# mir-group/nequip

Hardware: NVIDIA H100
Metric: atom-steps/sec (energy+forces) (higher is better)
Workload: dtype f32

## Files before the change

include/nqb.h:

```cpp
#ifndef NQB_H
#define NQB_H

#include <stddef.h>
#include <stdint.h>

#ifdef __cplusplus
extern "C" {
#endif

typedef struct CUstream_st* nqb_stream_t;
typedef struct nqb_plan nqb_plan;

typedef struct nqb_irrep {
  int32_t mul;
  int32_t l;
  int32_t p;
} nqb_irrep;

typedef struct nqb_instruction {
  int32_t i_in1;
  int32_t i_in2;
  int32_t i_out;
} nqb_instruction;

enum { NQB_F32 = 0, NQB_F64 = 1 };

int nqb_abi_version(void);
const char* nqb_last_error(void);

int nqb_plan_create(const nqb_irrep* in1, int n_in1, const nqb_irrep* in2, int n_in2,
                    const nqb_irrep* out, int n_out, const nqb_instruction* ins, int n_ins,
                    const char* spec_lib_path, nqb_plan** plan);
void nqb_plan_destroy(nqb_plan* plan);
int nqb_plan_dims(const nqb_plan* plan, int* d_in, int* s_dim, int* weight_numel, int* d_out);
int nqb_plan_signature(const nqb_plan* plan, char* buf, int buflen);

int nqb_csr_check_sorted(const int64_t* keys, int64_t E, int32_t* flag_dev, nqb_stream_t st);
int nqb_csr_from_sorted(const int64_t* sorted_keys, int64_t E, int64_t N, int64_t* row_ptr ,
                        nqb_stream_t st);

int nqb_tp_scatter_fwd(const nqb_plan* plan, int dtype, const void* x, const void* y, const void* w,
                       const int64_t* row_ptr, const int64_t* perm, const int64_t* src, int64_t N,
                       int64_t E, void* out, nqb_stream_t st);

int nqb_tp_scatter_bwd(const nqb_plan* plan, int dtype, const void* x, const void* y, const void* w,
                       const int64_t* row_ptr, const int64_t* perm, const int64_t* src,
                       const void* grad_out, int64_t N, int64_t E, void* grad_x, void* grad_y,
                       void* grad_w, int deterministic,
                       nqb_stream_t st);
int nqb_tp_scatter_gy_slices(const nqb_plan* plan, int dtype);
int nqb_segment_sum(int dtype, const void* rows , int D, const int64_t* perm, const int64_t* seg_ptr ,
                    int64_t N, void* out , nqb_stream_t st);

int nqb_sh_fwd(int lmax, const double* vec, int64_t E, int out_dtype, void* y, nqb_stream_t st);
int nqb_sh_bwd(int lmax, const double* vec, int64_t E, int out_dtype, const void* grad_y,
               double* grad_vec, nqb_stream_t st);

int nqb_tp_fused_slices(const nqb_plan* plan);
int nqb_tp_fused_fwd(const nqb_plan* plan, const float* x, const float* y, const float* h, int64_t ldh, int K,
                     const float* w2_prepared, const int64_t* row_ptr, const int64_t* src, int64_t N, int64_t E,
                     float* out, float* w_out, const int32_t* slice_cta0, int nctas, nqb_stream_t st);

int nqb_edge_embed_fwd(int lmax, int num_bessel, double r_max, double poly_p, double prefactor,
                       const double* pos, const int64_t* edge_index, const double* shift,
                       const double* cell, int64_t N, int64_t E, int out_dtype, double* vec, void* y,
                       void* emb, nqb_stream_t st);
int nqb_edge_embed_bwd(int lmax, int num_bessel, double r_max, double poly_p, double prefactor,
                       const double* vec, const int64_t* edge_index, int64_t N, int64_t E,
                       int out_dtype, const void* grad_y, const void* grad_emb, double* grad_pos,
                       double* grad_vec, nqb_stream_t st);

int nqb_zbl_fwd(const double* pos, const int64_t* edge_index, const double* shift, const double* cell,
                const double* vec, const int64_t* types, const double* table, int T, const int64_t* row_ptr,
                const int64_t* perm, int64_t N, int64_t E, double r_max, double poly_p, int cutoff_f32,
                double* e_atom, nqb_stream_t st);
int nqb_zbl_bwd(const double* pos, const int64_t* edge_index, const double* shift, const double* cell,
                const double* vec, const int64_t* types, const double* table, int T, int64_t N, int64_t E,
                double r_max, double poly_p, int cutoff_f32, const double* grad_e_atom, double* grad_pos,
                double* grad_vec, nqb_stream_t st);

int nqb_nl_bin(const double* pos, int64_t N, const double* cell_host, const double* inv_host, const int* pbc,
               const int* nbins, const int* search, const double* lo, const double* width, double r_max,
               double* wpos , int32_t* base , int64_t* bin , int32_t* cidx ,
               nqb_stream_t st);
int nqb_nl_count(int64_t N, const double* cell_host, const double* inv_host, const int* pbc, const int* nbins,
                 const int* search, double r_max, const double* wpos, const int32_t* cidx, const int64_t* order,
                 const int64_t* bin_start, int64_t* counts , nqb_stream_t st);
int nqb_nl_fill(int64_t N, int64_t E, const double* cell_host, const double* inv_host, const int* pbc, const int* nbins,
                const int* search, double r_max, const double* wpos, const int32_t* cidx, const int32_t* base,
                const int64_t* order, const int64_t* bin_start, const int64_t* row_ptr ,
                int64_t* edge_index , double* shifts , nqb_stream_t st);
int nqb_nl_pad(int64_t N, int64_t capacity, const int64_t* row_ptr, int64_t* row_ptr_pad, int64_t* num_edges,
               int32_t* overflow, nqb_stream_t st);
int nqb_nl_fill_capacity(int64_t N, int64_t capacity, const double* cell_host, const double* inv_host, const int* pbc,
                         const int* nbins, const int* search, double r_max, const double* wpos, const int32_t* cidx,
                         const int32_t* base, const int64_t* order, const int64_t* bin_start,
                         const int64_t* row_ptr_pad , const int32_t* overflow ,
                         const double* pad_shift_host, int64_t* edge_index ,
                         double* shifts , nqb_stream_t st);
int64_t nqb_nl_params_bytes(void);
int nqb_nl_params_pack(const double* cell_host, const double* inv_host, const int* pbc, const int* nbins,
                       const int* search, double r_max, const double* pad_shift_host, void* out_host);
int nqb_nl_bin_dp(const double* pos, int64_t N, const void* params_dev, double* wpos ,
                  int32_t* base , int64_t* bin , int32_t* cidx , nqb_stream_t st);
int nqb_nl_count_dp(int64_t N, const void* params_dev, const double* wpos, const int32_t* cidx, const int64_t* order,
                    const int64_t* bin_start, int64_t* counts , nqb_stream_t st);
int nqb_nl_fill_capacity_dp(int64_t N, int64_t capacity, const void* params_dev, const double* wpos,
                            const int32_t* cidx, const int32_t* base, const int64_t* order, const int64_t* bin_start,
                            const int64_t* row_ptr_pad , const int32_t* overflow ,
                            int64_t* edge_index , double* shifts ,
                            nqb_stream_t st);

int nqb_mlp_hidden_fwd(const float* emb, const float* W1s, int64_t E, int num_bessel, int hidden, float* h,
                       nqb_stream_t st);
int nqb_mlp_hidden_bwd(const float* emb, const float* W1s, const float* grad_h, int64_t E, int num_bessel,
                       int hidden, float* grad_emb, nqb_stream_t st);

int64_t nqb_gemm_prepared_floats(int K, int N);
int nqb_gemm_prepare(const float* B, int64_t ldb, int K, int N, int transposed, float scale, float* prepared,
                     nqb_stream_t st);
int nqb_gemm_grouped(const void* descs_dev, int ndesc, int ntiles_total, const int32_t* tile_ctas_dev,
                     int sched_ctas, const float* a_base, const float* prepared_base, float* c_base,
                     const float* rowscale_base, int64_t rs_ld, int64_t M, nqb_stream_t st);
int nqb_gemm_grouped_act(const void* descs_dev, int ndesc, int ntiles_total, const int32_t* tile_ctas_dev,
                         int sched_ctas, const float* a_base, const float* prepared_base, float* c_base,
                         const float* rowscale_base, int64_t rs_ld, int64_t M, float* aux_base, nqb_stream_t st);

int nqb_gate_fwd(int dtype, const void* x, int64_t N, int d_in, int d_out, const int32_t* src,
                 const int32_t* gate, const int32_t* kind, void* out, nqb_stream_t st);
int nqb_gate_bwd(int dtype, const void* x, const void* grad_out, int64_t N, int d_in, int d_out,
                 const int32_t* tab, void* grad_x, nqb_stream_t st);

int64_t nqb_launch_count(void);

#ifdef __cplusplus
}
#endif
#endif
```

nequip_b200/_capi.py:

```python
from __future__ import annotations

import ctypes as C
import os
from typing import Optional

from . import build

_lib: Optional[C.CDLL] = None


class NqbIrrep(C.Structure):
    _fields_ = [("mul", C.c_int32), ("l", C.c_int32), ("p", C.c_int32)]


class NqbInstruction(C.Structure):
    _fields_ = [("i_in1", C.c_int32), ("i_in2", C.c_int32), ("i_out", C.c_int32)]


_vp, _i64, _i32, _dbl = C.c_void_p, C.c_int64, C.c_int, C.c_double

SIGNATURES = {
    "nqb_abi_version": (_i32, []),
    "nqb_last_error": (C.c_char_p, []),
    "nqb_launch_count": (_i64, []),
    "nqb_plan_create": (
        _i32,
        [C.POINTER(NqbIrrep), _i32, C.POINTER(NqbIrrep), _i32, C.POINTER(NqbIrrep), _i32,
         C.POINTER(NqbInstruction), _i32, C.c_char_p, C.POINTER(_vp)],
    ),
    "nqb_plan_destroy": (None, [_vp]),
    "nqb_plan_dims": (_i32, [_vp, C.POINTER(_i32), C.POINTER(_i32), C.POINTER(_i32), C.POINTER(_i32)]),
    "nqb_plan_signature": (_i32, [_vp, C.c_char_p, _i32]),
    "nqb_csr_check_sorted": (_i32, [_vp, _i64, _vp, _vp]),
    "nqb_csr_from_sorted": (_i32, [_vp, _i64, _i64, _vp, _vp]),
    "nqb_tp_scatter_fwd": (_i32, [_vp, _i32, _vp, _vp, _vp, _vp, _vp, _vp, _i64, _i64, _vp, _vp]),
    "nqb_tp_scatter_bwd": (
        _i32, [_vp, _i32, _vp, _vp, _vp, _vp, _vp, _vp, _vp, _i64, _i64, _vp, _vp, _vp, _i32, _vp]),
    "nqb_tp_fused_slices": (_i32, [_vp]),
    "nqb_tp_fused_fwd": (_i32, [_vp, _vp, _vp, _vp, _i64, _i32, _vp, _vp, _vp, _i64, _i64, _vp, _vp, _vp, _i32, _vp]),
    "nqb_tp_scatter_gy_slices": (_i32, [_vp, _i32]),
    "nqb_segment_sum": (_i32, [_i32, _vp, _i32, _vp, _vp, _i64, _vp, _vp]),
    "nqb_nl_bin": (_i32, [_vp, _i64, _vp, _vp, _vp, _vp, _vp, _vp, _vp, _dbl, _vp, _vp, _vp, _vp, _vp]),
    "nqb_nl_count": (_i32, [_i64, _vp, _vp, _vp, _vp, _vp, _dbl, _vp, _vp, _vp, _vp, _vp, _vp]),
    "nqb_nl_fill": (_i32, [_i64, _i64, _vp, _vp, _vp, _vp, _vp, _dbl, _vp, _vp, _vp, _vp, _vp, _vp, _vp, _vp, _vp]),
    "nqb_nl_pad": (_i32, [_i64, _i64, _vp, _vp, _vp, _vp, _vp]),
    "nqb_nl_fill_capacity": (
        _i32, [_i64, _i64, _vp, _vp, _vp, _vp, _vp, _dbl, _vp, _vp, _vp, _vp, _vp, _vp, _vp, _vp, _vp, _vp, _vp]),
    "nqb_nl_params_bytes": (_i64, []),
    "nqb_nl_params_pack": (_i32, [_vp, _vp, _vp, _vp, _vp, _dbl, _vp, _vp]),
    "nqb_nl_bin_dp": (_i32, [_vp, _i64, _vp, _vp, _vp, _vp, _vp, _vp]),
    "nqb_nl_count_dp": (_i32, [_i64, _vp, _vp, _vp, _vp, _vp, _vp, _vp]),
    "nqb_nl_fill_capacity_dp": (_i32, [_i64, _i64, _vp, _vp, _vp, _vp, _vp, _vp, _vp, _vp, _vp, _vp, _vp]),
    "nqb_sh_fwd": (_i32, [_i32, _vp, _i64, _i32, _vp, _vp]),
    "nqb_sh_bwd": (_i32, [_i32, _vp, _i64, _i32, _vp, _vp, _vp]),
    "nqb_edge_embed_fwd": (
        _i32, [_i32, _i32, _dbl, _dbl, _dbl, _vp, _vp, _vp, _vp, _i64, _i64, _i32, _vp, _vp, _vp, _vp]),
    "nqb_edge_embed_bwd": (
        _i32, [_i32, _i32, _dbl, _dbl, _dbl, _vp, _vp, _i64, _i64, _i32, _vp, _vp, _vp, _vp, _vp]),
    "nqb_zbl_fwd": (
        _i32, [_vp, _vp, _vp, _vp, _vp, _vp, _vp, _i32, _vp, _vp, _i64, _i64, _dbl, _dbl, _i32, _vp, _vp]),
    "nqb_zbl_bwd": (
        _i32, [_vp, _vp, _vp, _vp, _vp, _vp, _vp, _i32, _i64, _i64, _dbl, _dbl, _i32, _vp, _vp, _vp, _vp]),
    "nqb_mlp_hidden_fwd": (_i32, [_vp, _vp, _i64, _i32, _i32, _vp, _vp]),
    "nqb_mlp_hidden_bwd": (_i32, [_vp, _vp, _vp, _i64, _i32, _i32, _vp, _vp]),
    "nqb_gemm_prepared_floats": (_i64, [_i32, _i32]),
    "nqb_gemm_prepare": (_i32, [_vp, _i64, _i32, _i32, _i32, C.c_float, _vp, _vp]),
    "nqb_gate_fwd": (_i32, [_i32, _vp, _i64, _i32, _i32, _vp, _vp, _vp, _vp, _vp]),
    "nqb_gate_bwd": (_i32, [_i32, _vp, _vp, _i64, _i32, _i32, _vp, _vp, _vp]),
    "nqb_gemm_grouped": (_i32, [_vp, _i32, _i32, _vp, _i32, _vp, _vp, _vp, _vp, _i64, _i64, _vp]),
    "nqb_gemm_grouped_act": (_i32, [_vp, _i32, _i32, _vp, _i32, _vp, _vp, _vp, _vp, _i64, _i64, _vp, _vp]),
}


def lib() -> C.CDLL:
    global _lib
    if _lib is None:
        path = os.environ.get("NQB_RUNTIME_LIB") or build.ensure_runtime()
        L = C.CDLL(path, mode=C.RTLD_GLOBAL)
        for name, (res, args) in SIGNATURES.items():
            fn = getattr(L, name)
            fn.restype = res
            fn.argtypes = args
        if L.nqb_abi_version() != 2:
            raise RuntimeError("libnqb.so ABI version mismatch")
        _lib = L
    return _lib


def check(rc: int, what: str = "") -> None:
    if rc != 0:
        msg = lib().nqb_last_error()
        raise RuntimeError(f"libnqb {what}: {msg.decode() if msg else 'error'} (rc={rc})")


def launch_count() -> int:
    return int(lib().nqb_launch_count())
```

nequip_b200/csrc/nqb_gemm.cu:

```cuda
#include <cuda_runtime.h>
#include <stdint.h>
#include <stdio.h>

#include "../../include/nqb.h"
#include "nqb_tc.cuh"

namespace {

constexpr int TM = 128;
constexpr int TN = 128;
constexpr int KC = 32;
constexpr int MW = 64;
constexpr int NWG = TM / MW;
constexpr int DEPTH = 2;
constexpr int RAW = DEPTH + 1;
constexpr int NLO = 2;
constexpr int BSLOTS = 4;
constexpr int SEG = 320 / KC;
constexpr int NTHREADS = NWG * 128;
constexpr int BLOCK_FLOATS = 2 * TN * KC;

struct GemmDesc {
  int64_t a_off, c_off, b_off, rs_off;
  int64_t lda, ldc, K, N;
  int64_t kchunks, ntiles, tile0, flags;
};

struct Smem {
  float b[BSLOTS][BLOCK_FLOATS];
  float araw[NWG][RAW][MW * KC];
  float alo[NWG][NLO][MW * KC];
  uint64_t b_full[BSLOTS], b_empty[BSLOTS];
};

__device__ __forceinline__ const GemmDesc* find_desc(const GemmDesc* d, int nd, int q) {
  int i = 0;
  while (i + 1 < nd && d[i + 1].tile0 <= q) ++i;
  return d + i;
}

struct Sched {
  int q, q_step, nq_total;
  int64_t m_start, m_step;
  __device__ Sched(int b, int G, int T, const int32_t* tile_ctas, int sched_ctas) {
    nq_total = T;
    if (tile_ctas != nullptr && G == sched_ctas) {
      q = T; q_step = T; m_start = 0; m_step = 1;
      for (int t = 0; t < T; ++t) {
        const int c0 = tile_ctas[2 * t], n = tile_ctas[2 * t + 1];
        if (b >= c0 && b < c0 + n) { q = t; m_start = b - c0; m_step = n; break; }
      }
    } else if (T <= G) {
      const int R = G / T;
      q = (b < T * R) ? (b % T) : T;
      q_step = T;
      m_start = b / T;
      m_step = R;
    } else {
      q = b; q_step = G; m_start = 0; m_step = 1;
    }
  }
};

struct WorkQ {
  const GemmDesc* d;
  int nt, kchunks, K, ncols;
  bool resident;
};
__device__ __forceinline__ void decode_q(const GemmDesc* descs, int ndesc, int q, WorkQ& w) {
  w.d = find_desc(descs, ndesc, q);
  w.nt = q - (int)w.d->tile0;
  w.kchunks = (int)w.d->kchunks;
  w.K = (int)w.d->K;
  w.ncols = min(TN, (int)w.d->N - w.nt * TN);
  w.resident = w.kchunks <= BSLOTS;
}

__device__ __forceinline__ void bar_wg(int wg) { asm volatile("bar.sync %0, 128;" ::"r"(1 + wg) : "memory"); }

template <bool ACT>
__global__ void __launch_bounds__(NTHREADS, 1)
k_gemm3x(const GemmDesc* __restrict__ descs, int ndesc, int ntiles_total, const int32_t* __restrict__ tile_ctas,
         int sched_ctas, const float* __restrict__ a_base, const float* __restrict__ b_base, float* __restrict__ c_base,
         const float* __restrict__ rs_base, int64_t rs_ld, int64_t M, float* __restrict__ aux_base) {
  extern __shared__ __align__(1024) uint8_t smem_raw[];
  Smem& S = *reinterpret_cast<Smem*>(smem_raw);
  const int tid = threadIdx.x, wg = tid >> 7, warp = (tid >> 5) & 3, lane = tid & 31;
  const int64_t mtiles = (M + TM - 1) / TM;

  if (tid == 0) {
    for (int s = 0; s < BSLOTS; ++s) { mbar_init(&S.b_full[s], 1); mbar_init(&S.b_empty[s], NWG * 4); }
    fence_barrier_init();
  }
  __syncthreads();
  const Sched sch(blockIdx.x, gridDim.x, ntiles_total, tile_ctas, sched_ctas);

  const int r8 = lane & 7, kq = lane >> 3;
  const int my_off = (2 * warp) * (KC / 4 * 32) + kq * 32 + r8 * 4;
  int pq = sch.q, ph_ = 0, pnh = 1, pK = 0;
  int64_t pmt = sch.m_start, plda = 0;
  const float* pA = nullptr;
  bool pvalid = pq < sch.nq_total && sch.m_start < mtiles;
  auto open_q = [&]() {
    WorkQ w;
    decode_q(descs, ndesc, pq, w);
    pA = a_base + w.d->a_off;
    plda = w.d->lda;
    pK = w.K;
    pnh = w.kchunks;
  };
  if (pvalid) open_q();
  uint32_t n_issued = 0;
  auto issue = [&]() {
    if (pvalid) {
      float* dst = S.araw[wg][n_issued % RAW] + my_off;
#pragma unroll
      for (int g = 0; g < 2; ++g) {
        const int64_t m = pmt * TM + wg * MW + warp * 16 + g * 8 + r8;
#pragma unroll
        for (int kh = 0; kh < 2; ++kh) {
          const int k = ph_ * KC + (kh * 4 + kq) * 4;
          const bool in = m < M && k < pK;
          const int64_t off = in ? m * plda + k : 0;
          cp_async16(dst + g * (KC / 4 * 32) + kh * 128, pA + off, in ? 16u : 0u);
        }
      }
      if (++ph_ == pnh) {
        ph_ = 0;
        pmt += sch.m_step;
        if (pmt >= mtiles) {
          pmt = sch.m_start;
          pq += sch.q_step;
          pvalid = pq < sch.nq_total;
          if (pvalid) open_q();
        }
      }
    }
    ++n_issued;
    cp_async_commit();
  };
#pragma unroll 1
  for (int j = 0; j < DEPTH; ++j) issue();

  uint32_t bused = 0, bpar_ld = 0;
  auto load_slot = [&](int slot, const float* src, uint32_t bytes) {
    if ((bused >> slot) & 1) mbar_wait(&S.b_empty[slot], ((bpar_ld >> slot) & 1) ^ 1);
    mbar_expect_tx(&S.b_full[slot], 2 * bytes);
    bulk_g2s(S.b[slot], src, bytes, &S.b_full[slot]);
    bulk_g2s(S.b[slot] + TN * KC, src + TN * KC, bytes, &S.b_full[slot]);
    bused |= 1u << slot;
    bpar_ld ^= 1u << slot;
  };
  uint32_t bpar = 0;

  constexpr uint32_t SBO = (KC / 4) * 128, LBO = 128;
  constexpr uint32_t A_STAGE = (MW * KC * sizeof(float)) >> 4;
  constexpr uint32_t B_SLOT = (BLOCK_FLOATS * sizeof(float)) >> 4, B_LO = (TN * KC * sizeof(float)) >> 4;
  const uint64_t dR0 = make_desc(smem_u32(S.araw[wg][0]), LBO, SBO);
  const uint64_t dL0 = make_desc(smem_u32(S.alo[wg][0]), LBO, SBO);
  const uint64_t dB0 = make_desc(smem_u32(S.b[0]), LBO, SBO);
  const int r0 = warp * 16 + (lane >> 2), c0 = 2 * (lane & 3);
  float hh[64], xx[64], acc[64];
  uint32_t i = 0;

  for (int q = sch.q; q < sch.nq_total; q += sch.q_step) {
    WorkQ w;
    decode_q(descs, ndesc, q, w);
    if (sch.m_start >= mtiles) continue;
    const GemmDesc* d = w.d;
    const int nseg = (w.kchunks + SEG - 1) / SEG;
    const int64_t nmt = (mtiles - 1 - sch.m_start) / sch.m_step + 1;
    const int64_t nload = w.resident ? w.kchunks : nmt * w.kchunks;
    const uint32_t bytes = (uint32_t)TN * KC * sizeof(float);
    const float* B = b_base + d->b_off + (int64_t)w.nt * w.kchunks * BLOCK_FLOATS;
    if (tid == 0)
      for (int64_t c = 0; c < min((int64_t)BSLOTS, nload); ++c) load_slot((int)c, B + (c % w.kchunks) * BLOCK_FLOATS, bytes);
    int64_t x = 0, xr = 0;
    auto release = [&](int64_t y) {
      const int slot = (int)(y % BSLOTS);
      if (lane == 0) mbar_arrive(&S.b_empty[slot]);
      if (tid == 0 && y + BSLOTS < nload) load_slot(slot, B + ((y + BSLOTS) % w.kchunks) * BLOCK_FLOATS, bytes);
    };
    const bool reduce = (d->flags & 5) != 0, skipz = (d->flags & 2) != 0;
    const int64_t ldc = d->ldc;
    float* C = c_base + d->c_off + (int64_t)w.nt * TN;
    [[maybe_unused]] const int act = ACT ? (int)(d->flags >> 3) & 7 : 0;
    [[maybe_unused]] float* X = ACT && (act & 6) ? aux_base + d->c_off + (int64_t)w.nt * TN : nullptr;
    bool first_mt = true;
    for (int64_t mt = sch.m_start; mt < mtiles; mt += sch.m_step) {
      for (int seg = 0; seg < nseg; ++seg) {
        const int h1 = min(w.kchunks, (seg + 1) * SEG);
        for (int h = seg * SEG; h < h1; ++h, ++i) {
          cp_async_wait<DEPTH - 1>();
          const float* raw = S.araw[wg][i % RAW] + my_off;
          float* lo = S.alo[wg][i % NLO] + my_off;
#pragma unroll
          for (int g = 0; g < 2; ++g)
#pragma unroll
            for (int kh = 0; kh < 2; ++kh) {
              const float4 t = *reinterpret_cast<const float4*>(raw + g * (KC / 4 * 32) + kh * 128);
              *reinterpret_cast<float4*>(lo + g * (KC / 4 * 32) + kh * 128) =
                  make_float4(tf32_lo(t.x), tf32_lo(t.y), tf32_lo(t.z), tf32_lo(t.w));
            }
          fence_proxy_async();
          bar_wg(wg);
          uint32_t slot;
          if (w.resident) {
            slot = h;
            if (first_mt) { mbar_wait(&S.b_full[slot], (bpar >> slot) & 1); bpar ^= 1u << slot; }
          } else {
            slot = (uint32_t)(x++ % BSLOTS);
            mbar_wait(&S.b_full[slot], (bpar >> slot) & 1);
            bpar ^= 1u << slot;
          }
          const uint64_t a_hi = dR0 + (uint64_t)((i % RAW) * A_STAGE), a_lo = dL0 + (uint64_t)((i % NLO) * A_STAGE);
          const uint64_t b_hi = dB0 + (uint64_t)(slot * B_SLOT), b_lo = b_hi + B_LO;
          const uint32_t fresh = (h == seg * SEG);
          wgmma_fence();
#pragma unroll
          for (int ks = 0; ks < KC / 8; ++ks) wgmma_tf32_m64n128(hh, a_hi + ks * 16, b_hi + ks * 16, !(fresh && ks == 0));
#pragma unroll
          for (int ks = 0; ks < KC / 8; ++ks) wgmma_tf32_m64n128(xx, a_lo + ks * 16, b_hi + ks * 16, !(fresh && ks == 0));
#pragma unroll
          for (int ks = 0; ks < KC / 8; ++ks) wgmma_tf32_m64n128(xx, a_hi + ks * 16, b_lo + ks * 16, 1u);
          wgmma_commit();
          wgmma_wait<1>();
          if (xr + 1 < x) release(xr++);
          issue();
        }
        wgmma_wait<0>();
        if (xr < x) release(xr++);
        if (seg + 1 < nseg) {
#pragma unroll
          for (int j = 0; j < 64; ++j) acc[j] = (seg == 0 ? 0.f : acc[j]) + (hh[j] + xx[j]);
        } else {
#pragma unroll
          for (int j = 0; j < 64; ++j) hh[j] = (seg == 0) ? hh[j] + xx[j] : acc[j] + (hh[j] + xx[j]);
        }
      }
      const int64_t m0 = mt * TM + wg * MW + r0;
#pragma unroll
      for (int half = 0; half < 2; ++half) {
        const int64_t m = m0 + half * 8;
        float rs = 1.0f;
        if (d->rs_off >= 0) rs = (m < M) ? __ldg(rs_base + d->rs_off * rs_ld + m) : 0.f;
        if (m >= M || (skipz && rs == 0.f)) continue;
        float* crow = C + m * ldc + c0;
#pragma unroll
        for (int j = 0; j < TN / 8; ++j) {
          if (j * 8 + c0 < w.ncols) {
            float v0 = hh[4 * j + 2 * half] * rs, v1 = hh[4 * j + 2 * half + 1] * rs;
            if constexpr (ACT) {
              if (act != 0) {
                float* xp = X + m * ldc + c0 + j * 8;
                if (act & 4) {
                  const float2 p = *reinterpret_cast<const float2*>(xp);
                  const float s0 = sigmoid(p.x), s1 = sigmoid(p.y);
                  v0 *= s0 * fmaf(p.x, 1.0f - s0, 1.0f);
                  v1 *= s1 * fmaf(p.y, 1.0f - s1, 1.0f);
                } else {
                  if (act & 2) *reinterpret_cast<float2*>(xp) = make_float2(v0, v1);
                  if (act & 1) {
                    v0 *= sigmoid(v0);
                    v1 *= sigmoid(v1);
                  }
                }
              }
            }
            if (reduce)
              asm volatile("red.global.add.v2.f32 [%0], {%1, %2};" ::"l"(crow + j * 8), "f"(v0), "f"(v1) : "memory");
            else
              *reinterpret_cast<float2*>(crow + j * 8) = make_float2(v0, v1);
          }
        }
      }
      first_mt = false;
    }
    if (w.resident && lane == 0)
      for (int c = 0; c < w.kchunks; ++c) mbar_arrive(&S.b_empty[c]);
  }
  cp_async_wait<0>();
}

__global__ void k_gemm_prepare(const float* __restrict__ B, int64_t ldb, int K, int N, int transposed, float scale,
                               float* __restrict__ out, int kchunks, int ntiles) {
  const int64_t total = (int64_t)ntiles * kchunks * TN * KC;
  for (int64_t idx = (int64_t)blockIdx.x * blockDim.x + threadIdx.x; idx < total; idx += (int64_t)gridDim.x * blockDim.x) {
    const int kk = (int)(idx % KC);
    const int nn = (int)((idx / KC) % TN);
    const int64_t blk = idx / (KC * TN);
    const int c = (int)(blk % kchunks), j = (int)(blk / kchunks);
    const int k = c * KC + kk, n = j * TN + nn;
    float v = 0.f;
    if (k < K && n < N) v = (transposed ? B[(int64_t)n * ldb + k] : B[(int64_t)k * ldb + n]) * scale;
    const float hi = tf32_rn(v), lo = v - hi;
    float* tile = out + blk * BLOCK_FLOATS;
    const int off = canon_off(nn, kk, KC / 4);
    tile[off] = hi;
    tile[TN * KC + off] = lo;
  }
}

}

extern "C" int nqb_set_error(const char* msg);
extern "C" void nqb_count_launch(void);

static int gemm_device() {
  int dev = 0;
  cudaGetDevice(&dev);
  return dev & 63;
}
static int gemm_sm_count() {
  static int n[64] = {0};
  const int dev = gemm_device();
  if (n[dev] == 0) {
    cudaDeviceGetAttribute(&n[dev], cudaDevAttrMultiProcessorCount, dev);
    if (n[dev] <= 0) n[dev] = 132;
  }
  return n[dev];
}

extern "C" int64_t nqb_gemm_prepared_floats(int K, int N) {
  const int64_t kchunks = (K + KC - 1) / KC, ntiles = (N + TN - 1) / TN;
  return kchunks * ntiles * BLOCK_FLOATS;
}

extern "C" int nqb_gemm_prepare(const float* B, int64_t ldb, int K, int N, int transposed, float scale, float* prepared,
                                nqb_stream_t st) {
  if (!B || !prepared) return nqb_set_error("nqb_gemm_prepare: null pointer");
  if (K <= 0 || N <= 0) return nqb_set_error("nqb_gemm_prepare: bad shape");
  const int kchunks = (K + KC - 1) / KC, ntiles = (N + TN - 1) / TN;
  const int64_t total = (int64_t)ntiles * kchunks * TN * KC;
  int blocks = (int)((total + 255) / 256);
  if (blocks > 4096) blocks = 4096;
  k_gemm_prepare<<<blocks, 256, 0, (cudaStream_t)st>>>(B, ldb, K, N, transposed, scale, prepared, kchunks, ntiles);
  nqb_count_launch();
  cudaError_t e = cudaGetLastError();
  if (e != cudaSuccess) return nqb_set_error(cudaGetErrorString(e));
  return 0;
}

template <bool ACT>
static int gemm_grouped_launch(const char* who, const void* descs_dev, int ndesc, int ntiles_total,
                               const int32_t* tile_ctas_dev, int sched_ctas, const float* a_base,
                               const float* prepared_base, float* c_base, float* aux_base, const float* rowscale_base,
                               int64_t rs_ld, int64_t M, nqb_stream_t st) {
  auto fail = [&](const char* what) {
    char msg[160];
    snprintf(msg, sizeof(msg), "%s: %s", who, what);
    return nqb_set_error(msg);
  };
  if (ndesc <= 0 || ntiles_total <= 0) return fail("empty problem list");
  if (M < 0) return fail("negative M");
  if (M == 0) return 0;
  if (!descs_dev || !a_base || !prepared_base || !c_base) return fail("null pointer");
  if (ACT && !aux_base) return fail("aux_base is null (bit4 / bit5 problems store to or read from it)");
  if (((uintptr_t)a_base | (uintptr_t)prepared_base | (uintptr_t)c_base | (uintptr_t)aux_base) & 15)
    return fail(ACT ? "a_base, prepared_base, c_base and aux_base must be 16-byte aligned"
                    : "a_base, prepared_base and c_base must be 16-byte aligned");
  static bool attr_set[64] = {false};
  const int dev = gemm_device();
  if (!attr_set[dev]) {
    cudaError_t e = cudaFuncSetAttribute(k_gemm3x<ACT>, cudaFuncAttributeMaxDynamicSharedMemorySize, (int)sizeof(Smem) + 1024);
    if (e != cudaSuccess) return nqb_set_error(cudaGetErrorString(e));
    attr_set[dev] = true;
  }
  const int64_t nwork = ((M + TM - 1) / TM) * (int64_t)ntiles_total;
  int grid = (int)(nwork < gemm_sm_count() ? nwork : gemm_sm_count());
  if (tile_ctas_dev != nullptr && sched_ctas > 0 && sched_ctas <= gemm_sm_count()) grid = sched_ctas;
  else tile_ctas_dev = nullptr;
  k_gemm3x<ACT><<<grid, NTHREADS, sizeof(Smem) + 1024, (cudaStream_t)st>>>(
      (const GemmDesc*)descs_dev, ndesc, ntiles_total, tile_ctas_dev, sched_ctas, a_base, prepared_base, c_base,
      rowscale_base, rs_ld, M, aux_base);
  nqb_count_launch();
  cudaError_t e = cudaGetLastError();
  if (e != cudaSuccess) return nqb_set_error(cudaGetErrorString(e));
  return 0;
}

extern "C" int nqb_gemm_grouped(const void* descs_dev, int ndesc, int ntiles_total, const int32_t* tile_ctas_dev,
                                int sched_ctas, const float* a_base, const float* prepared_base, float* c_base,
                                const float* rowscale_base, int64_t rs_ld, int64_t M, nqb_stream_t st) {
  return gemm_grouped_launch<false>("nqb_gemm_grouped", descs_dev, ndesc, ntiles_total, tile_ctas_dev, sched_ctas,
                                    a_base, prepared_base, c_base, nullptr, rowscale_base, rs_ld, M, st);
}

extern "C" int nqb_gemm_grouped_act(const void* descs_dev, int ndesc, int ntiles_total, const int32_t* tile_ctas_dev,
                                    int sched_ctas, const float* a_base, const float* prepared_base, float* c_base,
                                    const float* rowscale_base, int64_t rs_ld, int64_t M, float* aux_base,
                                    nqb_stream_t st) {
  return gemm_grouped_launch<true>("nqb_gemm_grouped_act", descs_dev, ndesc, ntiles_total, tile_ctas_dev, sched_ctas,
                                   a_base, prepared_base, c_base, aux_base, rowscale_base, rs_ld, M, st);
}
```

nequip_b200/csrc/nqb_mlp.cu:

```cuda
#include <cuda_runtime.h>
#include <stdint.h>

#include "../../include/nqb.h"
#include "nqb_tc.cuh"

namespace {

constexpr int H = 128;
constexpr int NB = 8;

struct Basis8 { float4 a, b; };
__device__ __forceinline__ Basis8 load_basis(const float* __restrict__ emb, int64_t e, int64_t E) {
  Basis8 r;
  if (e < E) {
    r.a = __ldg(reinterpret_cast<const float4*>(emb + e * NB));
    r.b = __ldg(reinterpret_cast<const float4*>(emb + e * NB + 4));
  } else {
    r.a = make_float4(0.f, 0.f, 0.f, 0.f);
    r.b = r.a;
  }
  return r;
}
__device__ __forceinline__ void bcast_basis(const Basis8& mine, int j, float (&x)[NB]) {
  x[0] = __shfl_sync(0xffffffffu, mine.a.x, j); x[1] = __shfl_sync(0xffffffffu, mine.a.y, j);
  x[2] = __shfl_sync(0xffffffffu, mine.a.z, j); x[3] = __shfl_sync(0xffffffffu, mine.a.w, j);
  x[4] = __shfl_sync(0xffffffffu, mine.b.x, j); x[5] = __shfl_sync(0xffffffffu, mine.b.y, j);
  x[6] = __shfl_sync(0xffffffffu, mine.b.z, j); x[7] = __shfl_sync(0xffffffffu, mine.b.w, j);
}
__device__ __forceinline__ void preact4(const float (&x)[NB], const float2 (&w01)[NB], const float2 (&w23)[NB],
                                        float2& p01, float2& p23) {
  p01 = make_float2(0.f, 0.f);
  p23 = p01;
#pragma unroll
  for (int k = 0; k < NB; ++k) {
    const float2 xx = make_float2(x[k], x[k]);
    p01 = fma2_rn(xx, w01[k], p01);
    p23 = fma2_rn(xx, w23[k], p23);
  }
}

__global__ void __launch_bounds__(256) k_hidden_fwd(const float* __restrict__ emb, const float* __restrict__ W1s,
                                                    int64_t E, float* __restrict__ h) {
  const int lane = threadIdx.x & 31, m0 = lane * 4;
  float2 w01[NB], w23[NB];
#pragma unroll
  for (int k = 0; k < NB; ++k) {
    const float4 t = __ldg(reinterpret_cast<const float4*>(W1s + k * H + m0));
    w01[k] = make_float2(t.x, t.y);
    w23[k] = make_float2(t.z, t.w);
  }
  const int64_t nwarps = (int64_t)gridDim.x * (blockDim.x >> 5);
  const int64_t nbatch = (E + 31) >> 5;
  int64_t b = (int64_t)blockIdx.x * (blockDim.x >> 5) + (threadIdx.x >> 5);
  Basis8 cur = load_basis(emb, b * 32 + lane, b < nbatch ? E : 0);
  for (; b < nbatch; b += nwarps) {
    const int64_t bn = b + nwarps;
    const Basis8 nxt = load_basis(emb, bn * 32 + lane, bn < nbatch ? E : 0);
    const int64_t e0 = b * 32;
    const int cnt = (int)((E - e0) < 32 ? (E - e0) : 32);
    float* hrow = h + e0 * H + m0;
#pragma unroll 2
    for (int j = 0; j < cnt; ++j) {
      float x[NB];
      bcast_basis(cur, j, x);
      float2 p01, p23;
      preact4(x, w01, w23, p01, p23);
      float4 o;
      o.x = p01.x * sigmoid(p01.x);
      o.y = p01.y * sigmoid(p01.y);
      o.z = p23.x * sigmoid(p23.x);
      o.w = p23.y * sigmoid(p23.y);
      __stcs(reinterpret_cast<float4*>(hrow + (int64_t)j * H), o);
    }
    cur = nxt;
  }
}

__global__ void __launch_bounds__(256) k_hidden_bwd(const float* __restrict__ emb, const float* __restrict__ W1s,
                                                    const float* __restrict__ gh, int64_t E, float* __restrict__ gemb) {
  const int lane = threadIdx.x & 31, m0 = lane * 4;
  float2 w01[NB], w23[NB];
#pragma unroll
  for (int k = 0; k < NB; ++k) {
    const float4 t = __ldg(reinterpret_cast<const float4*>(W1s + k * H + m0));
    w01[k] = make_float2(t.x, t.y);
    w23[k] = make_float2(t.z, t.w);
  }
  const int64_t nwarps = (int64_t)gridDim.x * (blockDim.x >> 5);
  const int64_t nbatch = (E + 31) >> 5;
  int64_t b = (int64_t)blockIdx.x * (blockDim.x >> 5) + (threadIdx.x >> 5);
  Basis8 cur = load_basis(emb, b * 32 + lane, b < nbatch ? E : 0);
  for (; b < nbatch; b += nwarps) {
    const int64_t bn = b + nwarps;
    const Basis8 nxt = load_basis(emb, bn * 32 + lane, bn < nbatch ? E : 0);
    const int64_t e0 = b * 32;
    const int cnt = (int)((E - e0) < 32 ? (E - e0) : 32);
    const float* grow = gh + e0 * H + m0;
#pragma unroll 1
    for (int j0 = 0; j0 < cnt; j0 += 4) {
      float4 g[4];
#pragma unroll
      for (int u = 0; u < 4; ++u)
        g[u] = (j0 + u < cnt) ? __ldcs(reinterpret_cast<const float4*>(grow + (int64_t)(j0 + u) * H))
                              : make_float4(0.f, 0.f, 0.f, 0.f);
      float v[32];
#pragma unroll
      for (int u = 0; u < 4; ++u) {
        float x[NB];
        bcast_basis(cur, (j0 + u) & 31, x);
        float2 p01, p23;
        preact4(x, w01, w23, p01, p23);
        const float s0 = sigmoid(p01.x), s1 = sigmoid(p01.y), s2 = sigmoid(p23.x), s3 = sigmoid(p23.y);
        const float2 gp01 = make_float2(g[u].x * (s0 * fmaf(p01.x, 1.0f - s0, 1.0f)), g[u].y * (s1 * fmaf(p01.y, 1.0f - s1, 1.0f)));
        const float2 gp23 = make_float2(g[u].z * (s2 * fmaf(p23.x, 1.0f - s2, 1.0f)), g[u].w * (s3 * fmaf(p23.y, 1.0f - s3, 1.0f)));
#pragma unroll
        for (int k = 0; k < NB; ++k) {
          const float2 t = fma2_rn(gp23, w23[k], fmul2_rn(gp01, w01[k]));
          v[u * 8 + k] = t.x + t.y;
        }
      }
#define NQB_HALVE(O, C)                                                        \
  {                                                                            \
    const bool up = (lane & (O)) != 0;                                         \
    _Pragma("unroll") for (int j = 0; j < (C); ++j) {                          \
      const float mine = up ? v[j + (C)] : v[j];                               \
      const float theirs = up ? v[j] : v[j + (C)];                             \
      v[j] = mine + __shfl_xor_sync(0xffffffffu, theirs, (O));                 \
    }                                                                          \
  }
      NQB_HALVE(16, 16)
      NQB_HALVE(8, 8)
      NQB_HALVE(4, 4)
      NQB_HALVE(2, 2)
      NQB_HALVE(1, 1)
#undef NQB_HALVE
      if (j0 + (lane >> 3) < cnt) gemb[(e0 + j0) * NB + lane] = v[0];
    }
    cur = nxt;
  }
}

}

extern "C" int nqb_set_error(const char* msg);
extern "C" void nqb_count_launch(void);

template <typename K>
static unsigned hidden_grid(K kernel, int which, int64_t E) {
  static int ctas_dev[2][64] = {{0}, {0}};
  int dev = 0;
  cudaGetDevice(&dev);
  dev &= 63;
  if (ctas_dev[which][dev] == 0) {
    int sms = 0, occ = 0;
    cudaDeviceGetAttribute(&sms, cudaDevAttrMultiProcessorCount, dev);
    if (cudaOccupancyMaxActiveBlocksPerMultiprocessor(&occ, kernel, 256, 0) != cudaSuccess || occ <= 0) occ = 2;
    ctas_dev[which][dev] = (sms > 0 ? sms : 132) * occ;
  }
  const int64_t need = (((E + 31) >> 5) + 7) / 8;
  return (unsigned)(need < ctas_dev[which][dev] ? need : ctas_dev[which][dev]);
}

extern "C" int nqb_mlp_hidden_fwd(const float* emb, const float* W1s, int64_t E, int num_bessel, int hidden, float* h,
                                  nqb_stream_t st) {
  if (num_bessel != NB || hidden != H) return nqb_set_error("nqb_mlp_hidden_fwd: only num_bessel=8, hidden=128 is built");
  if (E < 0) return nqb_set_error("nqb_mlp_hidden_fwd: negative size");
  if (E == 0) return 0;
  if (!emb || !W1s || !h) return nqb_set_error("nqb_mlp_hidden_fwd: null pointer");
  k_hidden_fwd<<<hidden_grid(k_hidden_fwd, 0, E), 256, 0, (cudaStream_t)st>>>(emb, W1s, E, h);
  nqb_count_launch();
  cudaError_t e = cudaGetLastError();
  if (e != cudaSuccess) return nqb_set_error(cudaGetErrorString(e));
  return 0;
}

extern "C" int nqb_mlp_hidden_bwd(const float* emb, const float* W1s, const float* grad_h, int64_t E, int num_bessel,
                                  int hidden, float* grad_emb, nqb_stream_t st) {
  if (num_bessel != NB || hidden != H) return nqb_set_error("nqb_mlp_hidden_bwd: only num_bessel=8, hidden=128 is built");
  if (E < 0) return nqb_set_error("nqb_mlp_hidden_bwd: negative size");
  if (E == 0) return 0;
  if (!emb || !W1s || !grad_h || !grad_emb) return nqb_set_error("nqb_mlp_hidden_bwd: null pointer");
  k_hidden_bwd<<<hidden_grid(k_hidden_bwd, 1, E), 256, 0, (cudaStream_t)st>>>(emb, W1s, grad_h, E, grad_emb);
  nqb_count_launch();
  cudaError_t e = cudaGetLastError();
  if (e != cudaSuccess) return nqb_set_error(cudaGetErrorString(e));
  return 0;
}
```

nequip_b200/nn/dense.py:

```python
from __future__ import annotations

from typing import List, Optional, Tuple

import torch

from .. import ops
from ..irreps import Irreps


def _aligned(*vals) -> bool:
    return all(v % 4 == 0 for v in vals)


class _GemmLinearFn(torch.autograd.Function):
    @staticmethod
    def forward(ctx, x, fwd: ops.GroupedGemm, bwd: ops.GroupedGemm, d_out: int, zero_out: bool, d_in: int, zero_in: bool,
                rowscale, out_init):
        M = x.shape[0]
        if out_init is not None:
            out = out_init
        else:
            out = (torch.zeros if zero_out else torch.empty)((M, d_out), dtype=x.dtype, device=x.device)
        fwd.run(x, out, M, rowscale)
        ctx.bwd, ctx.d_in, ctx.zero_in, ctx.rowscale = bwd, d_in, zero_in, rowscale
        ctx.has_init = out_init is not None
        if out_init is not None:
            ctx.mark_dirty(out_init)
        return out

    @staticmethod
    @torch.autograd.function.once_differentiable
    def backward(ctx, gout):
        gout = gout.contiguous()
        M = gout.shape[0]
        gx = (torch.zeros if ctx.zero_in else torch.empty)((M, ctx.d_in), dtype=gout.dtype, device=gout.device)
        ctx.bwd.run(gout, gx, M, ctx.rowscale)
        return gx, None, None, None, None, None, None, None, (gout if ctx.has_init else None)


class IrrepsLinearGemm:

    def __init__(self, lin, device, extra_scale: float = 1.0, row_scaled: bool = False):
        fin, fout = lin.irreps_in, lin.irreps_out
        rs = 0 if row_scaled else -1
        self.row_scaled = row_scaled
        in_off, out_off = fin.offsets(), fout.offsets()
        self.d_in, self.d_out = fin.dim, fout.dim
        fwd: List[ops.GemmProblem] = []
        bwd: List[ops.GemmProblem] = []
        n_out = {o: sum(1 for (_, o2, _, _) in lin.instr if o2 == o) for o in range(len(fout))}
        n_in = {i: sum(1 for (i2, _, _, _) in lin.instr if i2 == i) for i in range(len(fin))}
        for (i, o, off, pw) in lin.instr:
            mi, ir = fin[i]
            mo = fout[o][0]
            W = lin.weight.detach()[off: off + mi * mo].view(mi, mo)
            for c in range(ir.dim):
                a_off, c_off = in_off[i] + c * mi, out_off[o] + c * mo
                fwd.append(ops.GemmProblem(a_off, self.d_in, c_off, self.d_out, W, scale=pw * extra_scale,
                                           atomic=n_out[o] > 1, rs_off=rs))
                bwd.append(ops.GemmProblem(c_off, self.d_out, a_off, self.d_in, W, scale=pw * extra_scale, transposed=True,
                                           atomic=n_in[i] > 1, rs_off=rs))
        self.zero_out = any(n != 1 for n in n_out.values())
        self.zero_in = any(n != 1 for n in n_in.values())
        self.fwd = ops.GroupedGemm(fwd, device)
        self.bwd = ops.GroupedGemm(bwd, device)

    @staticmethod
    def supported(lin) -> bool:
        muls = [m for m, _ in lin.irreps_in] + [m for m, _ in lin.irreps_out]
        return lin.layout == "ir_mul" and all(m % 4 == 0 for m in muls) and lin.weight.dtype == torch.float32

    def __call__(self, x, rowscale=None):
        if self.row_scaled != (rowscale is not None):
            raise ValueError("IrrepsLinearGemm: rowscale must be given exactly when built with row_scaled=True")
        return _GemmLinearFn.apply(x.contiguous(), self.fwd, self.bwd, self.d_out, self.zero_out, self.d_in, self.zero_in,
                                   rowscale, None)


class SelfConnectionGemm:

    def __init__(self, sc, type_table: torch.Tensor, device):
        fin, fout = sc.irreps_in, sc.irreps_out
        in_off, out_off = fin.offsets(), fout.offsets()
        self.d_in, self.d_out = fin.dim, fout.dim
        self.T = type_table.shape[0]
        fwd: List[ops.GemmProblem] = []
        bwd: List[ops.GemmProblem] = []
        tt = type_table.detach()
        for (i, o, off, pw) in sc.instr:
            mi, ir = fin[i]
            mo = fout[o][0]
            W = sc.weight.detach()[off: off + mi * sc.num_attr * mo].view(mi, sc.num_attr, mo)
            weff = torch.einsum("uvw,tv->tuw", W, tt)
            for t in range(self.T):
                for c in range(ir.dim):
                    a_off, c_off = in_off[i] + c * mi, out_off[o] + c * mo
                    multi_o = sum(1 for (_, o2, _, _) in sc.instr if o2 == o) > 1
                    fwd.append(ops.GemmProblem(a_off, self.d_in, c_off, self.d_out, weff[t].contiguous(), scale=pw,
                                               accumulate=not multi_o, atomic=multi_o, rs_off=t, skip_zero_rows=True))
                    multi_i = sum(1 for (i2, _, _, _) in sc.instr if i2 == i) > 1
                    bwd.append(ops.GemmProblem(c_off, self.d_out, a_off, self.d_in, weff[t].contiguous(), scale=pw,
                                               transposed=True, accumulate=not multi_i, atomic=multi_i, rs_off=t,
                                               skip_zero_rows=True))
        self.zero_in = True
        self.fwd = ops.GroupedGemm(fwd, device)
        self.bwd = ops.GroupedGemm(bwd, device)

    @staticmethod
    def supported(sc) -> bool:
        muls = [m for m, _ in sc.irreps_in] + [m for m, _ in sc.irreps_out]
        return sc.layout == "ir_mul" and all(m % 4 == 0 for m in muls) and sc.weight.dtype == torch.float32

    def __call__(self, x, types, base):
        onehot_t = torch.nn.functional.one_hot(types, self.T).to(x.dtype).t().contiguous()
        return _GemmLinearFn.apply(x.contiguous(), self.fwd, self.bwd, self.d_out, False, self.d_in, self.zero_in,
                                   onehot_t, base)


class _RadialMLPGemmFn(torch.autograd.Function):
    @staticmethod
    def forward(ctx, emb, mlp: "RadialMLPGemm", need_bwd: bool):
        E = emb.shape[0]
        out = torch.empty((E, mlp.W), dtype=emb.dtype, device=emb.device)
        pre = [] if need_bwd else None
        mlp.fwd.run(mlp.hidden(emb, pre), out, E)
        ctx.mlp = mlp
        if need_bwd:
            ctx.save_for_backward(emb, *pre)
        return out

    @staticmethod
    @torch.autograd.function.once_differentiable
    def backward(ctx, gw):
        emb, *pre = ctx.saved_tensors
        return ctx.mlp.grad_emb(emb, gw, pre), None, None


class RadialMLPGemm:

    def __init__(self, first, last, device, middle=()):
        self.w1s = (first.weight.detach() * first.alpha).contiguous()
        self.W = last.weight.shape[1]
        plan = self.plan(first, last, middle)
        self._hidden_kernel = plan["hidden_kernel"]

        def gemm(p):
            return ops.GroupedGemm([p], device)

        self.fwd = gemm(plan["fwd"])
        self.bwd = gemm(plan["bwd"])
        self._hidden = [(gemm(save), gemm(plain), save.B.shape[1]) for save, plain in plan["hidden"]]
        self._chain = [(self.bwd if p is plan["bwd"] else gemm(p), width, pre) for p, width, pre in plan["chain"]]

    @staticmethod
    def uses_hidden_kernel(first) -> bool:
        return tuple(first.weight.shape) == (8, 128)

    @classmethod
    def plan(cls, first, last, middle=()):

        def prob(lin, act="none", transposed=False):
            k, n = lin.weight.shape
            lda, ldc = (n, k) if transposed else (k, n)
            return ops.GemmProblem(0, lda, 0, ldc, lin.weight.detach(), scale=float(lin.alpha), transposed=transposed,
                                   act=act)

        layers = [first, *middle, last]
        kernel = cls.uses_hidden_kernel(first)
        skip = 1 if kernel else 0
        bwd = prob(last, transposed=True)
        chain = []
        for i in range(len(layers) - 1, 0, -1):
            pre = i - 1 - skip
            if pre >= 0:
                p = prob(layers[i], "silu_grad", True)
            else:
                p = bwd if i == len(layers) - 1 else prob(layers[i], transposed=True)
            chain.append((p, layers[i].weight.shape[0], pre if pre >= 0 else None))
        if not kernel:
            chain.append((prob(first, transposed=True), first.weight.shape[0], None))
        return dict(hidden_kernel=kernel, hidden=[(prob(l, "silu_save"), prob(l, "silu")) for l in layers[skip:-1]],
                    fwd=prob(last), bwd=bwd, chain=chain)

    @staticmethod
    def supported(first, last, dtype, middle=()) -> bool:
        dims = [first.weight.shape[0]] + [l.weight.shape[1] for l in (first, *middle, last)]
        return dtype == torch.float32 and all(d % 4 == 0 for d in dims)

    def hidden(self, emb, pre: Optional[list] = None):
        E = emb.shape[0]
        x = emb
        if self._hidden_kernel:
            x = torch.empty((E, self.w1s.shape[1]), dtype=emb.dtype, device=emb.device)
            ops.mlp_hidden_fwd(emb, self.w1s, x)
        for save, plain, width in self._hidden:
            h = torch.empty((E, width), dtype=emb.dtype, device=emb.device)
            if pre is None:
                plain.run(x, h, E)
            else:
                p = torch.empty((E, width), dtype=emb.dtype, device=emb.device)
                save.run(x, h, E, aux=p)
                pre.append(p)
            x = h
        return x

    def grad_emb(self, emb, gw, pre=()):
        E = emb.shape[0]
        g = gw.contiguous()
        for gemm, width, k in self._chain:
            out = torch.empty((E, width), dtype=g.dtype, device=g.device)
            gemm.run(g, out, E, aux=None if k is None else pre[k])
            g = out
        if self._hidden_kernel:
            gemb = torch.empty_like(emb)
            ops.mlp_hidden_bwd(emb, self.w1s, g, gemb)
            return gemb
        return g

    def __call__(self, emb):
        return _RadialMLPGemmFn.apply(emb.contiguous(), self, torch.is_grad_enabled() and emb.requires_grad)


class _FusedRadialTPFn(torch.autograd.Function):

    @staticmethod
    def forward(ctx, emb, x, y, edge_src, mod: "FusedRadialTP", csr, need_emb_grad: bool):
        pre = [] if need_emb_grad else None
        h = mod.mlp.hidden(emb, pre)
        need_bwd = any(ctx.needs_input_grad[:3])
        out, w = ops.tp_fused_fwd(mod.fw, x, y, h, edge_src, csr, want_w=need_bwd)
        ctx.mod, ctx.csr = mod, csr
        if need_bwd:
            ctx.save_for_backward(emb, x, y, w, edge_src, *(pre or ()))
        return out

    @staticmethod
    @torch.autograd.function.once_differentiable
    def backward(ctx, gout):
        emb, x, y, w, edge_src, *pre = ctx.saved_tensors
        mod = ctx.mod
        gx, gy, gw = ops.tp_scatter_bwd_raw(mod.plan, x, y, w, edge_src, ctx.csr, gout, need_x=ctx.needs_input_grad[1])
        gemb = mod.mlp.grad_emb(emb, gw, pre) if ctx.needs_input_grad[0] else None
        return gemb, gx, (gy if ctx.needs_input_grad[2] else None), None, None, None, None


class FusedRadialTP:

    def __init__(self, mlp: RadialMLPGemm, lin2, plan: ops.TPPlan, device):
        self.plan = plan
        self.mlp = mlp
        self.fw = ops.FusedTPWeights(plan, lin2.weight.detach(), float(lin2.alpha), device)

    @staticmethod
    def supported(lin1, lin2, plan: ops.TPPlan, dtype) -> bool:
        hid, W = lin2.weight.shape
        if dtype != torch.float32 or hid > 128 or hid % 8 or W != plan.weight_numel or W % 4:
            return False
        return int(ops._capi.lib().nqb_tp_fused_slices(plan.handle)) > 0

    def __call__(self, emb, x, y, edge_dst, edge_src):
        csr = ops.csr_cache.get(edge_dst.long().contiguous() if edge_dst.dtype != torch.int64 else edge_dst, x.shape[0])
        if csr.perm is not None:
            return None
        return _FusedRadialTPFn.apply(emb.contiguous(), x.contiguous(), y.contiguous(), edge_src.long().contiguous(), self, csr,
                                      torch.is_grad_enabled() and emb.requires_grad)
```

nequip_b200/nn/model.py:

```python
from __future__ import annotations

import math
from typing import Dict, List, Optional, Sequence, Tuple, Union

import torch

from .. import ops
from ..irreps import Irrep, Irreps, build_tp_instructions, tp_path_exists
from .pair import ZBL, ZBL_TARGET, parse_pair_potential
from .tp_scatter import B200TensorProductScatter

C_SILU = 1.6791767923989418
C_TANH = 1.5937334472592692

POSITIONS_KEY = "pos"
EDGE_INDEX_KEY = "edge_index"
EDGE_CELL_SHIFT_KEY = "edge_cell_shift"
CELL_KEY = "cell"
ATOM_TYPE_KEY = "atom_types"
TOTAL_ENERGY_KEY = "total_energy"
PER_ATOM_ENERGY_KEY = "atomic_energy"
FORCE_KEY = "forces"
STRESS_KEY = "stress"
VIRIAL_KEY = "virial"
EDGE_VECTORS_KEY = "edge_vectors"
EDGE_FORCE_KEY = "edge_forces"
BATCH_KEY = "batch"
BATCH_PTR_KEY = "ptr"
NUM_NODES_KEY = "num_atoms"


def feature_widths(l_max: int, num_features) -> List[int]:
    if isinstance(num_features, int):
        return [num_features] * (l_max + 1)
    widths = [int(f) for f in num_features]
    if len(widths) != l_max + 1:
        raise ValueError(f"num_features: expected an int or l_max + 1 = {l_max + 1} widths, got {list(num_features)}")
    return widths


def hidden_irreps(l_max: int, num_features, parity: bool) -> Irreps:
    widths = feature_widths(l_max, num_features)
    items = []
    for l in range(l_max + 1):
        ps = (1, -1) if parity else ((1,) if l % 2 == 0 else (-1,))
        for p in ps:
            items.append((widths[l], Irrep(l, p)))
    return Irreps(items)


def gate_irreps(prev: Irreps, edge_attr: Irreps, hidden: Irreps):
    scalars = Irreps([(mul, ir) for mul, ir in hidden if ir.l == 0 and tp_path_exists(prev, edge_attr, ir)])
    gated = Irreps([(mul, ir) for mul, ir in hidden if ir.l > 0 and tp_path_exists(prev, edge_attr, ir)])
    gate_ir = Irrep(0, 1) if tp_path_exists(prev, edge_attr, Irrep(0, 1)) else Irrep(0, -1)
    gates = Irreps([(mul, gate_ir) for mul, _ in gated])
    conv_out = (scalars + gates + gated).simplify()
    gated_out = Irreps([(mul, Irrep(ir.l, ir.p * gate_ir.p)) for mul, ir in gated])
    layer_out = scalars + gated_out
    return scalars, gates, gated, conv_out, layer_out


def layer_irreps(l_max: int, num_features, num_layers: int, parity: bool = True, type_embed_num_features=None):
    widths = feature_widths(l_max, num_features)
    f0 = type_embed_num_features or widths[0]
    edge_attr = Irreps.spherical_harmonics(l_max)
    prev = Irreps([(f0, Irrep(0, 1))])
    hid = hidden_irreps(l_max, widths, parity)
    hiddens = [hid] * (num_layers - 1) + [Irreps([(widths[0], Irrep(0, 1))])]
    out = []
    for h in hiddens:
        scalars, gates, gated, conv_out, layer_out = gate_irreps(prev, edge_attr, h)
        out.append((prev, edge_attr, conv_out, (scalars, gates, gated)))
        prev = layer_out
    return out


class ScalarLinearLayer(torch.nn.Module):

    def __init__(self, in_features: int, out_features: int, alpha: float = 1.0):
        super().__init__()
        self.in_features, self.out_features = in_features, out_features
        self.register_buffer("alpha", torch.tensor(alpha), persistent=False)
        self.weight = torch.nn.Parameter(torch.empty((in_features, out_features)))
        torch.nn.init.uniform_(self.weight, -math.sqrt(3), math.sqrt(3))

    def forward(self, x):
        return torch.mm(x, self.weight * self.alpha)


class ScalarMLPFunction(torch.nn.Module):

    def __init__(self, input_dim: int, output_dim: int, hidden_layers_depth: int = 0,
                 hidden_layers_width: Optional[int] = None, nonlinearity: Optional[str] = "silu"):
        super().__init__()
        dims = [input_dim] + hidden_layers_depth * [hidden_layers_width] + [output_dim]
        self.dims = dims
        layers: List[torch.nn.Module] = []
        nl = len(dims) - 1
        for layer, (h_in, h_out) in enumerate(zip(dims, dims[1:])):
            gain = 1.0 if nonlinearity is None or layer == 0 else math.sqrt(2)
            layers.append(ScalarLinearLayer(h_in, h_out, alpha=gain / math.sqrt(h_in)))
            if layer != nl - 1 and nonlinearity is not None:
                layers.append(torch.nn.SiLU())
        self.mlp = torch.nn.Sequential(*layers)

    def forward(self, x):
        return self.mlp(x)


class Linear(torch.nn.Module):

    def __init__(self, irreps_in, irreps_out, layout: str = "mul_ir"):
        super().__init__()
        self.layout = layout
        self.irreps_in, self.irreps_out = Irreps(irreps_in), Irreps(irreps_out)
        self.instr: List[Tuple[int, int, int, float]] = []
        off = 0
        pairs = [
            (i, o)
            for i, (_, ir_i) in enumerate(self.irreps_in)
            for o, (_, ir_o) in enumerate(self.irreps_out)
            if ir_i == ir_o
        ]
        for (i, o) in pairs:
            fan = sum(self.irreps_in[i2][0] for (i2, o2) in pairs if o2 == o)
            self.instr.append((i, o, off, 1.0 / math.sqrt(fan)))
            off += self.irreps_in[i][0] * self.irreps_out[o][0]
        self.weight_numel = off
        self.weight = torch.nn.Parameter(torch.randn(off))
        self._in_sl, self._out_sl = self.irreps_in.slices(), self.irreps_out.slices()

    def forward(self, x):
        N = x.shape[0]
        outs: List[Optional[torch.Tensor]] = [None] * len(self.irreps_out)
        for (i, o, off, pw) in self.instr:
            mi, ir = self.irreps_in[i]
            mo = self.irreps_out[o][0]
            W = self.weight[off: off + mi * mo].view(mi, mo) * pw
            if self.layout == "ir_mul":
                r = torch.matmul(x[:, self._in_sl[i]].reshape(N * ir.dim, mi), W).reshape(N, ir.dim * mo)
            else:
                xi = x[:, self._in_sl[i]].reshape(N, mi, ir.dim)
                r = torch.matmul(xi.transpose(1, 2), W).transpose(1, 2).reshape(N, mo * ir.dim)
            outs[o] = r if outs[o] is None else outs[o] + r
        for o, (mo, ir) in enumerate(self.irreps_out):
            if outs[o] is None:
                outs[o] = x.new_zeros(N, mo * ir.dim)
        return torch.cat(outs, dim=1)


class SelfConnection(torch.nn.Module):

    def __init__(self, irreps_in, num_attr: int, irreps_out, layout: str = "mul_ir"):
        super().__init__()
        self.layout = layout
        self.irreps_in, self.irreps_out, self.num_attr = Irreps(irreps_in), Irreps(irreps_out), num_attr
        pairs = [
            (i, o)
            for i, (_, ir_i) in enumerate(self.irreps_in)
            for o, (_, ir_o) in enumerate(self.irreps_out)
            if ir_i == ir_o
        ]
        self.instr: List[Tuple[int, int, int, float]] = []
        off = 0
        for (i, o) in pairs:
            fan = sum(self.irreps_in[i2][0] * num_attr for (i2, o2) in pairs if o2 == o)
            self.instr.append((i, o, off, 1.0 / math.sqrt(fan)))
            off += self.irreps_in[i][0] * num_attr * self.irreps_out[o][0]
        self.weight_numel = off
        self.weight = torch.nn.Parameter(torch.randn(off))
        self._in_sl = self.irreps_in.slices()

    def forward(self, x, node_attrs, types=None, type_table=None):
        N = x.shape[0]
        outs: List[Optional[torch.Tensor]] = [None] * len(self.irreps_out)
        fast = types is not None and type_table is not None
        if fast:
            T = type_table.shape[0]
            onehot = torch.nn.functional.one_hot(types, T).to(x.dtype)
        for (i, o, off, pw) in self.instr:
            mi, ir = self.irreps_in[i]
            mo = self.irreps_out[o][0]
            W = self.weight[off: off + mi * self.num_attr * mo].view(mi, self.num_attr, mo)
            if self.layout == "ir_mul":
                xk = x[:, self._in_sl[i]].reshape(N, ir.dim, mi)
                if fast:
                    weff = torch.einsum("uvw,tv->tuw", W, type_table).reshape(T * mi, mo) * pw
                    xe = (onehot.view(N, 1, T, 1) * xk.unsqueeze(2)).reshape(N * ir.dim, T * mi)
                    r = torch.matmul(xe, weff).reshape(N, ir.dim * mo)
                else:
                    r = pw * torch.einsum("uvw,nku,nv->nkw", W, xk, node_attrs).reshape(N, ir.dim * mo)
                outs[o] = r if outs[o] is None else outs[o] + r
                continue
            xi = x[:, self._in_sl[i]].reshape(N, mi, ir.dim)
            if fast:
                weff = torch.einsum("uvw,tv->tuw", W, type_table).reshape(T * mi, mo) * pw
                xe = (onehot.view(N, 1, T, 1) * xi.transpose(1, 2).unsqueeze(2)).reshape(N, ir.dim, T * mi)
                r = torch.matmul(xe, weff).transpose(1, 2).reshape(N, mo * ir.dim)
            else:
                r = pw * torch.einsum("uvw,nuk,nv->nwk", W, xi, node_attrs).reshape(N, mo * ir.dim)
            outs[o] = r if outs[o] is None else outs[o] + r
        for o, (mo, ir) in enumerate(self.irreps_out):
            if outs[o] is None:
                outs[o] = x.new_zeros(N, mo * ir.dim)
        return torch.cat(outs, dim=1)


class Gate(torch.nn.Module):

    def __init__(self, irreps_scalars, irreps_gates, irreps_gated, layout: str = "mul_ir"):
        super().__init__()
        self.layout = layout
        self.irreps_scalars, self.irreps_gates, self.irreps_gated = (
            Irreps(irreps_scalars), Irreps(irreps_gates), Irreps(irreps_gated))
        self.irreps_in = self.irreps_scalars + self.irreps_gates + self.irreps_gated
        gp = self.irreps_gates[0][1].p if len(self.irreps_gates) else 1
        self.irreps_out = self.irreps_scalars + Irreps([(m, Irrep(ir.l, ir.p * gp)) for m, ir in self.irreps_gated])
        self.use_fused = True
        self._tabs = None

    @staticmethod
    def _act(x, p: int):
        return torch.nn.functional.silu(x) * C_SILU if p == 1 else torch.tanh(x) * C_TANH

    def forward(self, x):
        if x.is_cuda and self.use_fused:
            key = (x.device, self.layout)
            if self._tabs is None or self._tabs[0] != key:
                self._tabs = (key, ops.GateTables(self.irreps_scalars, self.irreps_gates, self.irreps_gated,
                                                  self.layout, x.device))
            return ops.gate(x, self._tabs[1])
        N = x.shape[0]
        ns, ng = self.irreps_scalars.dim, self.irreps_gates.dim
        parts = []
        off = 0
        for mul, ir in self.irreps_scalars:
            parts.append(self._act(x[:, off: off + mul], ir.p))
            off += mul
        if len(self.irreps_gated):
            gates = []
            goff = ns
            for mul, ir in self.irreps_gates:
                gates.append(self._act(x[:, goff: goff + mul], ir.p))
                goff += mul
            gates = torch.cat(gates, dim=1)
            off = ns + ng
            g0 = 0
            for mul, ir in self.irreps_gated:
                if self.layout == "ir_mul":
                    ch = x[:, off: off + mul * ir.dim].reshape(N, ir.dim, mul)
                    parts.append((ch * gates[:, g0: g0 + mul].unsqueeze(1)).reshape(N, mul * ir.dim))
                else:
                    ch = x[:, off: off + mul * ir.dim].reshape(N, mul, ir.dim)
                    parts.append((ch * gates[:, g0: g0 + mul].unsqueeze(-1)).reshape(N, mul * ir.dim))
                off += mul * ir.dim
                g0 += mul
        return torch.cat(parts, dim=1)


class InteractionBlock(torch.nn.Module):

    def __init__(self, feature_irreps_in, irreps_edge_attr, feature_irreps_out, num_edge_embed: int,
                 num_node_attrs: int, radial_mlp_depth: int, radial_mlp_width: int, use_sc: bool,
                 avg_num_neighbors: float, is_first_layer: bool = False, layout: str = "mul_ir"):
        super().__init__()
        self.is_first_layer = is_first_layer
        self.layout = layout
        fin, fe, fout = Irreps(feature_irreps_in), Irreps(irreps_edge_attr), Irreps(feature_irreps_out)
        self.feature_irreps_in, self.irreps_edge_attr, self.feature_irreps_out = fin, fe, fout
        ann = [float(avg_num_neighbors)] if isinstance(avg_num_neighbors, (int, float)) else [float(v) for v in avg_num_neighbors]
        self.register_buffer("norm_const", torch.tensor([1.0 / math.sqrt(v) for v in ann]).reshape(-1, 1), persistent=False)
        self.norm_shortcut = len(ann) == 1
        self.linear_1 = Linear(fin, fin, layout)
        irreps_mid, instructions = build_tp_instructions(fin, fe, fout)
        self.irreps_mid, self.instructions = irreps_mid, instructions
        self.tp_scatter = B200TensorProductScatter(fin, fe, irreps_mid, instructions, layout=layout)
        self.edge_mlp = ScalarMLPFunction(num_edge_embed, self.tp_scatter.weight_numel,
                                          hidden_layers_depth=radial_mlp_depth,
                                          hidden_layers_width=radial_mlp_width, nonlinearity="silu")
        self.linear_2 = Linear(irreps_mid.simplify(), fout, layout)
        self.sc = SelfConnection(fin, num_node_attrs, fout, layout) if use_sc else None
        self.use_tensor_cores = True
        self.use_fused_radial_tp = "auto"
        self._fused_choice = None
        self.strict_fast_path = False
        self._tc_cache = None

    def _edge_weights(self, edge_embedding):
        return self.edge_mlp(edge_embedding)

    def _use_fused(self, tc, edge_embedding, x, edge_attrs, edge_index) -> bool:
        mode = self.use_fused_radial_tp
        if mode is True or mode is False:
            return mode
        if self._fused_choice is None:
            if torch.cuda.is_current_stream_capturing():
                return False
            with torch.no_grad():
                def t(fn):
                    fn()
                    torch.cuda.synchronize()
                    e0, e1 = torch.cuda.Event(enable_timing=True), torch.cuda.Event(enable_timing=True)
                    e0.record()
                    for _ in range(2):
                        fn()
                    e1.record()
                    torch.cuda.synchronize()
                    return e0.elapsed_time(e1) / 2

                xd, yd, ed = x.detach(), edge_attrs.detach(), edge_embedding.detach()
                tf = t(lambda: tc["fused"](ed, xd, yd, edge_index[0], edge_index[1]))
                tu = t(lambda: self.tp_scatter(x=xd, edge_attr=yd, edge_weight=tc["mlp"](ed), edge_dst=edge_index[0],
                                               edge_src=edge_index[1]))
            self._fused_choice = bool(tf < tu)
            self.fused_timing_ms = {"fused": tf, "unfused": tu}
        return self._fused_choice

    def _note_fallback(self, reason: str):
        if getattr(self, "strict_fast_path", False):
            raise RuntimeError(f"nequip_b200 InteractionBlock: tensor-core fast path unavailable ({reason}) and "
                               "strict_fast_path=True")
        seen = self.__dict__.setdefault("_fallback_seen", set())
        if reason not in seen:
            seen.add(reason)
            import warnings

            warnings.warn(f"nequip_b200 InteractionBlock: dense blocks run through torch.matmul (cuBLAS), not the "
                          f"wgmma kernels: {reason}", RuntimeWarning, stacklevel=3)

    def forward(self, x, node_attrs, edge_attrs, edge_embedding, edge_index, types=None, type_table=None,
                n_own: Optional[int] = None, halo=None):
        if n_own is not None and not self.is_first_layer:
            x = x[:n_own]
            node_attrs = node_attrs[:n_own]
            types = None if types is None else types[:n_own]
        tc = self._tensor_core_blocks(x, types, type_table)
        if tc is not None:
            x_in = x
            x = tc["lin1"](x) if self.norm_shortcut else tc["lin1"](x, self.norm_const.view(-1)[types].view(1, -1).contiguous())
            if halo is not None and not self.is_first_layer:
                x = halo(x)
            if tc["fused"] is not None and self._use_fused(tc, edge_embedding, x, edge_attrs, edge_index):
                y = tc["fused"](edge_embedding, x, edge_attrs, edge_index[0], edge_index[1])
                if y is not None:
                    x = y
                    if n_own is not None:
                        x = x[:n_own]
                    x = tc["lin2"](x)
                    if tc["sc"] is not None:
                        x = tc["sc"](x_in, types, x)
                    return x
            if tc["mlp"] is not None:
                w = tc["mlp"](edge_embedding)
            else:
                self._note_fallback("radial MLP shape not supported by the grouped GEMM (needs at least one hidden "
                                    "layer, num_bessels and widths multiples of 4)")
                w = self._edge_weights(edge_embedding)
            x = self.tp_scatter(x=x, edge_attr=edge_attrs, edge_weight=w, edge_dst=edge_index[0], edge_src=edge_index[1])
            if n_own is not None:
                x = x[:n_own]
            x = tc["lin2"](x)
            if tc["sc"] is not None:
                x = tc["sc"](x_in, types, x)
            return x
        sc = self.sc(x, node_attrs, types, type_table) if self.sc is not None else None
        x = self.linear_1(x)
        x = x * (self.norm_const.view(()) if self.norm_shortcut else self.norm_const[types])
        if halo is not None and not self.is_first_layer:
            x = halo(x)
        w = self._edge_weights(edge_embedding)
        x = self.tp_scatter(x=x, edge_attr=edge_attrs, edge_weight=w, edge_dst=edge_index[0], edge_src=edge_index[1])
        if n_own is not None:
            x = x[:n_own]
        x = self.linear_2(x)
        if sc is not None:
            x = x + sc
        return x

    def _tensor_core_blocks(self, x, types, type_table):
        from . import dense

        if not self.use_tensor_cores or not x.is_cuda:
            return None
        if x.dtype != torch.float32 or self.layout != "ir_mul":
            self._note_fallback(f"dtype {x.dtype} / layout {self.layout} (needs float32, ir_mul)")
            return None
        if any(p.requires_grad for p in self.parameters()) or (type_table is not None and type_table.requires_grad):
            self._note_fallback("parameters require grad (training); freeze them for the inference path")
            return None
        if (self.sc is not None or not self.norm_shortcut) and (types is None or type_table is None):
            self._note_fallback("self-connection / per-type normalisation need atom types + type table")
            return None
        key = tuple((p.data_ptr(), p._version) for p in self.parameters()) + (
            (type_table.data_ptr(), type_table._version) if type_table is not None else ())
        if self._tc_cache is not None and self._tc_cache[0] == key:
            if self._tc_cache[1] is None:
                self._note_fallback("a multiplicity is not a multiple of 4")
            return self._tc_cache[1]
        ok = dense.IrrepsLinearGemm.supported(self.linear_1) and dense.IrrepsLinearGemm.supported(self.linear_2)
        if self.sc is not None:
            ok = ok and dense.SelfConnectionGemm.supported(self.sc)
        if not ok:
            self._note_fallback("a multiplicity is not a multiple of 4")
            self._tc_cache = (key, None)
            return None
        dev = x.device
        lins = [m for m in self.edge_mlp.mlp if isinstance(m, ScalarLinearLayer)]
        mlp = fused = None
        if len(lins) >= 2 and dense.RadialMLPGemm.supported(lins[0], lins[-1], x.dtype, middle=lins[1:-1]):
            mlp = dense.RadialMLPGemm(lins[0], lins[-1], dev, middle=lins[1:-1])
            if dense.FusedRadialTP.supported(lins[0], lins[-1], self.tp_scatter._plan, x.dtype):
                fused = dense.FusedRadialTP(mlp, lins[-1], self.tp_scatter._plan, dev)
        blocks = dict(
            fused=fused,
            lin1=(dense.IrrepsLinearGemm(self.linear_1, dev, extra_scale=float(self.norm_const.view(-1)[0]))
                  if self.norm_shortcut else dense.IrrepsLinearGemm(self.linear_1, dev, row_scaled=True)),
            lin2=dense.IrrepsLinearGemm(self.linear_2, dev),
            sc=dense.SelfConnectionGemm(self.sc, type_table, dev) if self.sc is not None else None,
            mlp=mlp,
        )
        self._tc_cache = (key, blocks)
        return blocks


class ConvNetLayer(torch.nn.Module):

    def __init__(self, prev: Irreps, edge_attr: Irreps, hidden: Irreps, **conv_kwargs):
        super().__init__()
        scalars, gates, gated, conv_out, layer_out = gate_irreps(prev, edge_attr, hidden)
        self.equivariant_nonlin = Gate(scalars, gates, gated, conv_kwargs.get("layout", "mul_ir"))
        self.conv = InteractionBlock(prev, edge_attr, conv_out, **conv_kwargs)
        self.irreps_out = layer_out

    def forward(self, x, node_attrs, edge_attrs, edge_embedding, edge_index, types=None, type_table=None,
                n_own=None, halo=None):
        x = self.conv(x, node_attrs, edge_attrs, edge_embedding, edge_index, types, type_table, n_own, halo)
        return self.equivariant_nonlin(x)


NEQUIP_PRESETS: Dict[str, dict] = {
    "S": dict(num_layers=2, l_max=1, num_features=[128, 64]),
    "M": dict(num_layers=4, l_max=2, num_features=[128, 64, 32]),
    "L": dict(num_layers=6, l_max=3, num_features=[128, 64, 32, 32]),
    "XL": dict(num_layers=6, l_max=4, num_features=[320, 96, 64, 32, 32]),
}
NEQUIP_STANDARD_PRESET = dict(parity=False, type_embed_num_features=32, radial_mlp_depth=1, radial_mlp_width=128)


def preset_kwargs(name: str, **overrides) -> dict:
    key = name.upper()
    if key not in NEQUIP_PRESETS:
        raise ValueError(f"unknown preset {name!r}: expected one of {sorted(NEQUIP_PRESETS)}")
    return {**NEQUIP_STANDARD_PRESET, **NEQUIP_PRESETS[key], **overrides}


class NequIPEnergyModel(torch.nn.Module):

    def __init__(self, *, r_max: float, type_names: Sequence[str], num_layers: int = 4, l_max: int = 1,
                 parity: bool = True, num_features: Union[int, Sequence[int]] = 32,
                 type_embed_num_features: Optional[int] = None, radial_mlp_depth: int = 1,
                 radial_mlp_width: int = 128, num_bessels: int = 8, polynomial_cutoff_p: float = 6.0,
                 avg_num_neighbors: float = 1.0, per_type_energy_scales: Optional[Sequence[float]] = None,
                 per_type_energy_shifts: Optional[Sequence[float]] = None, model_dtype=torch.float32,
                 seed: int = 123, node_layout: str = "ir_mul", strict_fast_path: bool = False,
                 pair_potential: Optional[dict] = None):
        super().__init__()
        pair_spec = parse_pair_potential(pair_potential, len(type_names))
        widths = feature_widths(l_max, num_features)
        f_embed = int(type_embed_num_features) if type_embed_num_features is not None else widths[0]
        self.r_max, self.l_max, self.num_bessels, self.poly_p = float(r_max), l_max, num_bessels, float(polynomial_cutoff_p)
        self.model_dtype = model_dtype
        self.node_layout = node_layout
        self.config = dict(r_max=r_max, type_names=list(type_names), num_layers=num_layers, l_max=l_max, parity=parity,
                           num_features=num_features if isinstance(num_features, int) else widths,
                           type_embed_num_features=f_embed, radial_mlp_depth=radial_mlp_depth,
                           radial_mlp_width=radial_mlp_width, num_bessels=num_bessels,
                           polynomial_cutoff_p=polynomial_cutoff_p, avg_num_neighbors=avg_num_neighbors)
        prev_default = torch.get_default_dtype()
        torch.set_default_dtype(model_dtype)
        try:
            torch.manual_seed(seed)
            ntypes = len(type_names)
            if isinstance(avg_num_neighbors, dict):
                if set(avg_num_neighbors) != set(type_names):
                    raise ValueError("avg_num_neighbors: keys must be the type names")
                avg_num_neighbors = [float(avg_num_neighbors[k]) for k in type_names]
            elif not isinstance(avg_num_neighbors, (int, float)):
                avg_num_neighbors = [float(v) for v in avg_num_neighbors]
                if len(avg_num_neighbors) not in (1, ntypes):
                    raise ValueError(f"avg_num_neighbors: expected a scalar or {ntypes} values")
            self.config["avg_num_neighbors"] = avg_num_neighbors
            self.type_embed = torch.nn.Embedding(ntypes, f_embed)
            edge_attr = Irreps.spherical_harmonics(l_max)
            prev = Irreps([(f_embed, Irrep(0, 1))])
            hid = hidden_irreps(l_max, widths, parity)
            hiddens = [hid] * (num_layers - 1) + [Irreps([(widths[0], Irrep(0, 1))])]
            layers = []
            for li, h in enumerate(hiddens):
                layer = ConvNetLayer(prev, edge_attr, h, num_edge_embed=num_bessels, num_node_attrs=f_embed,
                                     radial_mlp_depth=radial_mlp_depth, radial_mlp_width=radial_mlp_width,
                                     use_sc=(li != 0), avg_num_neighbors=avg_num_neighbors,
                                     is_first_layer=(li == 0), layout=node_layout)
                layers.append(layer)
                prev = layer.irreps_out
            self.layers = torch.nn.ModuleList(layers)
            self.readout = ScalarMLPFunction(prev.dim, 1, hidden_layers_depth=0)
        finally:
            torch.set_default_dtype(prev_default)
        def table(v, what):
            if v is None:
                return torch.empty(0, dtype=torch.float64)
            t = torch.as_tensor(v, dtype=torch.float64).reshape(-1)
            if t.numel() == 1:
                t = t.expand(ntypes).clone()
            if t.numel() != ntypes:
                raise ValueError(f"{what}: expected a scalar or {ntypes} values (one per type), got {t.numel()}")
            return t.reshape(-1, 1)

        self.register_buffer("scales", table(per_type_energy_scales, "per_type_energy_scales"))
        self.register_buffer("shifts", table(per_type_energy_shifts, "per_type_energy_shifts"))
        self.pair_potential = None
        if pair_spec is not None:
            self.pair_potential = ZBL(type_names, model_dtype=model_dtype, **pair_spec)
            self.config["pair_potential"] = dict(_target_=ZBL_TARGET, **pair_spec)
        self.set_strict_fast_path(strict_fast_path)

    @classmethod
    def from_preset(cls, name: str, **kwargs) -> "NequIPEnergyModel":
        return cls(**preset_kwargs(name, **kwargs))

    def set_strict_fast_path(self, on: bool = True):
        for layer in self.layers:
            layer.conv.strict_fast_path = bool(on)
        return self

    @staticmethod
    def _reduce_energy(e_atom: torch.Tensor, data: Dict[str, torch.Tensor]) -> torch.Tensor:
        batch = data.get(BATCH_KEY)
        if batch is None:
            return e_atom.sum(dim=0, keepdim=True)
        if NUM_NODES_KEY in data:
            ng = int(data[NUM_NODES_KEY].numel())
        elif BATCH_PTR_KEY in data:
            ng = int(data[BATCH_PTR_KEY].numel()) - 1
        else:
            ng = int(batch.max().item()) + 1 if batch.numel() else 0
        out = torch.zeros((ng, 1), dtype=e_atom.dtype, device=e_atom.device)
        return out.index_add_(0, batch.view(-1).long(), e_atom)

    def energy(self, data: Dict[str, torch.Tensor]) -> Dict[str, torch.Tensor]:
        pos = data[POSITIONS_KEY]
        edge_index = data[EDGE_INDEX_KEY]
        types = data[ATOM_TYPE_KEY].view(-1)
        node_attrs = self.type_embed(types)
        x = node_attrs
        shift, cell = data.get(EDGE_CELL_SHIFT_KEY), data.get(CELL_KEY)
        if cell is None:
            shift = None
        pre = (2 * math.pi) / (self.r_max * self.r_max)
        sink = data.get("_edge_grad_sink")
        if EDGE_VECTORS_KEY in data:
            edge_attrs, edge_embedding = ops.edge_embed_from_vectors(
                data[EDGE_VECTORS_KEY], lmax=self.l_max, num_bessel=self.num_bessels, r_max=self.r_max,
                poly_p=self.poly_p, prefactor=pre, out_dtype=self.model_dtype)
        else:
            _vec, edge_attrs, edge_embedding = ops.edge_embed(
                pos, edge_index, shift, cell, lmax=self.l_max, num_bessel=self.num_bessels, r_max=self.r_max,
                poly_p=self.poly_p, prefactor=pre, out_dtype=self.model_dtype, edge_grad_sink=sink)
        for layer in self.layers:
            x = layer(x, node_attrs, edge_attrs, edge_embedding, edge_index, types, self.type_embed.weight)
        e_atom = self.readout(x).to(torch.float64)
        if self.scales.numel():
            e_atom = e_atom * self.scales[types]
        if self.shifts.numel():
            e_atom = e_atom + self.shifts[types]
        if self.pair_potential is not None:
            if EDGE_VECTORS_KEY in data:
                e_pair = self.pair_potential(types, edge_index, self.r_max, edge_vectors=data[EDGE_VECTORS_KEY])
            else:
                e_pair = self.pair_potential(types, edge_index, self.r_max, pos=pos, shift=shift, cell=cell,
                                             edge_grad_sink=sink)
            e_atom = e_atom + e_pair
        data[PER_ATOM_ENERGY_KEY] = e_atom
        data[TOTAL_ENERGY_KEY] = self._reduce_energy(e_atom, data)
        return data

    def energy_owned(self, data: Dict[str, torch.Tensor], n_own: int, halo) -> torch.Tensor:
        pos, edge_index = data[POSITIONS_KEY], data[EDGE_INDEX_KEY]
        types = data[ATOM_TYPE_KEY].view(-1)
        node_attrs = self.type_embed(types)
        x = node_attrs
        shift, cell = data.get(EDGE_CELL_SHIFT_KEY), data.get(CELL_KEY)
        if cell is None:
            shift = None
        _vec, edge_attrs, edge_embedding = ops.edge_embed(
            pos, edge_index, shift, cell, lmax=self.l_max, num_bessel=self.num_bessels, r_max=self.r_max,
            poly_p=self.poly_p, prefactor=(2 * math.pi) / (self.r_max * self.r_max), out_dtype=self.model_dtype)
        for layer in self.layers:
            x = layer(x, node_attrs, edge_attrs, edge_embedding, edge_index, types, self.type_embed.weight, n_own, halo)
        e_atom = self.readout(x).to(torch.float64)
        t_own = types[:n_own]
        if self.scales.numel():
            e_atom = e_atom * self.scales[t_own]
        if self.shifts.numel():
            e_atom = e_atom + self.shifts[t_own]
        if self.pair_potential is not None:
            e_atom = e_atom + self.pair_potential(types, edge_index, self.r_max, pos=pos, shift=shift, cell=cell)[:n_own]
        return e_atom

    def forward(self, data: Dict[str, torch.Tensor], compute_forces: bool = True,
                compute_stress: bool = False) -> Dict[str, torch.Tensor]:
        data = dict(data)
        if not compute_forces:
            return self.energy(data)
        if EDGE_VECTORS_KEY in data:
            with torch.enable_grad():
                vec = data[EDGE_VECTORS_KEY].detach().double().requires_grad_(True)
                data[EDGE_VECTORS_KEY] = vec
                data = self.energy(data)
                (g,) = torch.autograd.grad([data[TOTAL_ENERGY_KEY].sum()], [vec])
            data[EDGE_FORCE_KEY] = g
            data[EDGE_VECTORS_KEY] = vec.detach()
            data[TOTAL_ENERGY_KEY] = data[TOTAL_ENERGY_KEY].detach()
            data[PER_ATOM_ENERGY_KEY] = data[PER_ATOM_ENERGY_KEY].detach()
            return data
        if compute_stress and data.get(CELL_KEY) is None:
            raise ValueError("compute_stress needs a cell")
        pos = data[POSITIONS_KEY]
        sink = {} if compute_stress else None
        with torch.enable_grad():
            pos = pos.detach().requires_grad_(True)
            data[POSITIONS_KEY] = pos
            if sink is not None:
                data["_edge_grad_sink"] = sink
            data = self.energy(data)
            (g,) = torch.autograd.grad([data[TOTAL_ENERGY_KEY].sum()], [pos])
        data.pop("_edge_grad_sink", None)
        data[FORCE_KEY] = torch.neg(g)
        if sink is not None:
            g_edge = sink["edge_vector_grad"]
            if "pair_edge_vector_grad" in sink:
                g_edge = g_edge + sink["pair_edge_vector_grad"]
            v = torch.einsum("ea,eb->ab", sink["edge_vectors"], g_edge)
            v = 0.5 * (v + v.t())
            vol = torch.linalg.det(data[CELL_KEY].double().view(3, 3)).abs()
            data[STRESS_KEY] = (v / vol).view(1, 3, 3)
            data[VIRIAL_KEY] = torch.neg(v).view(1, 3, 3)
        data[POSITIONS_KEY] = pos.detach()
        data[TOTAL_ENERGY_KEY] = data[TOTAL_ENERGY_KEY].detach()
        data[PER_ATOM_ENERGY_KEY] = data[PER_ATOM_ENERGY_KEY].detach()
        return data
```

nequip_b200/ops.py:

```python
from __future__ import annotations

import ctypes as C
import os
import threading
from dataclasses import dataclass
from typing import Dict, List, Optional, Tuple

import torch

from . import _capi, build
from .codegen import GenOptions, TPSignature
from .irreps import Irreps

_DT = {torch.float32: 0, torch.float64: 1}


def _stream() -> int:
    return torch.cuda.current_stream().cuda_stream


def _ptr(t: Optional[torch.Tensor]) -> int:
    return 0 if t is None else t.data_ptr()


def _require_cuda(*ts: torch.Tensor):
    for t in ts:
        if t is not None and not t.is_cuda:
            raise RuntimeError(
                "nequip_b200 kernels run on CUDA (sm_90a) only; got a CPU tensor and there is no CPU fallback"
            )


class TPPlan:

    def __init__(self, irreps_in1, irreps_in2, irreps_out, instructions, opts: Optional[GenOptions] = None):
        self.sig = TPSignature(Irreps(irreps_in1), Irreps(irreps_in2), Irreps(irreps_out), list(instructions))
        self.opts = opts or GenOptions()
        self.spec_path = build.ensure_spec(self.sig, self.opts)
        L = _capi.lib()

        def arr(irr):
            a = (_capi.NqbIrrep * len(irr))()
            for i, (mul, ir) in enumerate(irr):
                a[i].mul, a[i].l, a[i].p = mul, ir.l, ir.p
            return a

        in1, in2, out = arr(self.sig.irreps_in1), arr(self.sig.irreps_in2), arr(self.sig.irreps_out)
        ins = (_capi.NqbInstruction * len(self.sig.instructions))()
        for i, (a, b, c) in enumerate(self.sig.instructions):
            ins[i].i_in1, ins[i].i_in2, ins[i].i_out = a, b, c
        h = C.c_void_p()
        _capi.check(
            L.nqb_plan_create(in1, len(in1), in2, len(in2), out, len(out), ins, len(ins),
                              self.spec_path.encode(), C.byref(h)),
            "nqb_plan_create",
        )
        self._h = h
        self.d_in, self.s_dim = self.sig.d_in, self.sig.s_dim
        self.weight_numel, self.d_out = self.sig.weight_numel, self.sig.d_out

    @property
    def handle(self) -> C.c_void_p:
        return self._h

    def __del__(self):
        try:
            if getattr(self, "_h", None):
                _capi.lib().nqb_plan_destroy(self._h)
                self._h = None
        except Exception:
            pass


_plans: Dict[str, TPPlan] = {}
_plans_lock = threading.Lock()


def get_plan(irreps_in1, irreps_in2, irreps_out, instructions, opts: Optional[GenOptions] = None) -> TPPlan:
    opts = opts or GenOptions()
    sig = TPSignature(Irreps(irreps_in1), Irreps(irreps_in2), Irreps(irreps_out), list(instructions))
    key = sig.canonical() + "|" + opts.tag()
    with _plans_lock:
        p = _plans.get(key)
        if p is None:
            p = TPPlan(irreps_in1, irreps_in2, irreps_out, instructions, opts)
            _plans[key] = p
        return p


@dataclass
class EdgeCSR:
    row_ptr: torch.Tensor
    perm: Optional[torch.Tensor]
    num_nodes: int
    num_edges: int


def build_csr(edge_dst: torch.Tensor, num_nodes: int, assume_sorted: Optional[bool] = None) -> EdgeCSR:
    _require_cuda(edge_dst)
    if edge_dst.dtype != torch.int64:
        edge_dst = edge_dst.long()
    edge_dst = edge_dst.contiguous()
    E = edge_dst.numel()
    L = _capi.lib()
    st = _stream()
    is_sorted = assume_sorted
    deferred = getattr(_sorted_tls, "flags", None)
    if deferred is None and _capture_flags and torch.cuda.is_current_stream_capturing():
        deferred = _capture_flags[-1]
    if is_sorted is None and deferred is not None:
        flag = torch.empty(1, dtype=torch.int32, device=edge_dst.device)
        _capi.check(L.nqb_csr_check_sorted(_ptr(edge_dst), E, _ptr(flag), st), "nqb_csr_check_sorted")
        deferred.append(flag)
        is_sorted = True
    if is_sorted is None:
        flag = torch.empty(1, dtype=torch.int32, device=edge_dst.device)
        _capi.check(L.nqb_csr_check_sorted(_ptr(edge_dst), E, _ptr(flag), st), "nqb_csr_check_sorted")
        is_sorted = bool(flag.item())
    perm = None
    keys = edge_dst
    if not is_sorted:
        keys, perm = torch.sort(edge_dst, stable=True)
        perm = perm.contiguous()
        keys = keys.contiguous()
    row_ptr = torch.empty(num_nodes + 1, dtype=torch.int64, device=edge_dst.device)
    _capi.check(L.nqb_csr_from_sorted(_ptr(keys), E, num_nodes, _ptr(row_ptr), st), "nqb_csr_from_sorted")
    return EdgeCSR(row_ptr, perm, num_nodes, E)


_sorted_tls = threading.local()
_capture_flags: List[List[torch.Tensor]] = []


class deferred_sorted_check:

    def __enter__(self):
        self.flags: List[torch.Tensor] = []
        self._prev = getattr(_sorted_tls, "flags", None)
        _sorted_tls.flags = self.flags
        _capture_flags.append(self.flags)
        return self

    def __exit__(self, *exc):
        _sorted_tls.flags = self._prev
        for k in range(len(_capture_flags) - 1, -1, -1):
            if _capture_flags[k] is self.flags:
                del _capture_flags[k]
                break
        return False


class _CSRCache:

    def __init__(self):
        self._tls = threading.local()

    def get(self, edge_dst: torch.Tensor, num_nodes: int) -> EdgeCSR:
        key = (edge_dst.data_ptr(), edge_dst.numel(), edge_dst._version, num_nodes, edge_dst.device)
        ent = getattr(self._tls, "ent", None)
        if ent is not None and ent[0] == key:
            return ent[1]
        csr = build_csr(edge_dst, num_nodes)
        self._tls.ent = (key, csr, edge_dst)
        return csr

    def clear(self):
        self._tls.ent = None


csr_cache = _CSRCache()


class _TPScatterFn(torch.autograd.Function):
    @staticmethod
    def forward(ctx, x, edge_attr, edge_weight, edge_src, plan: TPPlan, csr: EdgeCSR):
        L = _capi.lib()
        N, E = x.shape[0], edge_src.numel()
        out = torch.empty((N, plan.d_out), dtype=x.dtype, device=x.device)
        if N > 0:
            _capi.check(
                L.nqb_tp_scatter_fwd(plan.handle, _DT[x.dtype], _ptr(x), _ptr(edge_attr), _ptr(edge_weight),
                                     _ptr(csr.row_ptr), _ptr(csr.perm), _ptr(edge_src), N, E, _ptr(out), _stream()),
                "nqb_tp_scatter_fwd",
            )
        ctx.plan, ctx.csr = plan, csr
        ctx.save_for_backward(x, edge_attr, edge_weight, edge_src)
        return out

    @staticmethod
    @torch.autograd.function.once_differentiable
    def backward(ctx, gout):
        x, y, w, edge_src = ctx.saved_tensors
        gx, gy, gw = tp_scatter_bwd_raw(ctx.plan, x, y, w, edge_src, ctx.csr, gout, need_x=ctx.needs_input_grad[0])
        return gx, (gy if ctx.needs_input_grad[1] else None), (gw if ctx.needs_input_grad[2] else None), None, None, None


def tp_scatter(plan: TPPlan, x, edge_attr, edge_weight, edge_dst, edge_src, csr: Optional[EdgeCSR] = None):
    _require_cuda(x, edge_attr, edge_weight, edge_dst, edge_src)
    if x.dtype not in _DT:
        raise TypeError(f"nequip_b200.tp_scatter: unsupported dtype {x.dtype}")
    dt = x.dtype
    if x.dim() != 2 or x.shape[1] != plan.d_in:
        raise ValueError(f"x must be [N, {plan.d_in}], got {tuple(x.shape)}")
    E = edge_src.numel()
    if tuple(edge_attr.shape) != (E, plan.s_dim) or tuple(edge_weight.shape) != (E, plan.weight_numel):
        raise ValueError(
            f"edge_attr/edge_weight must be [{E}, {plan.s_dim}] / [{E}, {plan.weight_numel}], got "
            f"{tuple(edge_attr.shape)} / {tuple(edge_weight.shape)}"
        )
    if edge_dst.numel() != E:
        raise ValueError("edge_dst and edge_src differ in length")
    x = x.contiguous()
    y = edge_attr.to(dt).contiguous()
    w = edge_weight.to(dt).contiguous()
    src = edge_src.long().contiguous()
    if csr is None:
        csr = csr_cache.get(edge_dst.long().contiguous() if edge_dst.dtype != torch.int64 else edge_dst, x.shape[0])
    elif csr.num_nodes != x.shape[0] or csr.num_edges != E:
        raise ValueError("EdgeCSR does not match x / edge_index")
    return _TPScatterFn.apply(x, y, w, src, plan, csr)


class FusedTPWeights:

    def __init__(self, plan: TPPlan, W2: torch.Tensor, alpha2: float, device):
        from .codegen import TPGenerator

        L = _capi.lib()
        self.plan = plan
        lay = TPGenerator(plan.sig, plan.opts).fused_layout()
        nslice = int(L.nqb_tp_fused_slices(plan.handle))
        if lay is None or nslice == 0 or nslice != len(lay["slices"]):
            raise RuntimeError("FusedTPWeights: this signature has no fused kernel")
        K, W = int(W2.shape[0]), int(W2.shape[1])
        if W != plan.weight_numel or K > 128 or K % 8:
            raise ValueError(f"FusedTPWeights: W2 must be [K <= 128 (multiple of 8), {plan.weight_numel}], got {tuple(W2.shape)}")
        self.K, self.nslice = K, nslice
        cols = torch.tensor(lay["cols"], dtype=torch.long, device=device)
        W2d = W2.detach().to(device=device, dtype=torch.float32)
        Wp = torch.zeros((K, cols.numel()), dtype=torch.float32, device=device)
        ok = cols >= 0
        Wp[:, ok] = W2d[:, cols[ok]]
        self.prepared = self.prepare(Wp * float(alpha2), nslice)
        G = torch.cuda.get_device_properties(device).multi_processor_count
        self.cta0, self.nctas = self.split_grid(lay["cost"], G)
        self.cta0_dev = torch.tensor(self.cta0, dtype=torch.int32, device=device)

    @staticmethod
    def prepare(Wp: torch.Tensor, nslice: int) -> torch.Tensor:
        K = Wp.shape[0]
        wt = torch.zeros((nslice, 128, 128), dtype=torch.float32, device=Wp.device)
        wt[:, :, :K] = Wp.t().reshape(nslice, 128, K)
        bits = wt.view(torch.int32)
        hi = ((bits + 0x1000) & -0x2000).view(torch.float32)
        lo = wt - hi
        both = torch.stack([hi, lo], 1)
        both = both.reshape(nslice, 2, 16, 8, 32, 4).permute(0, 1, 2, 4, 3, 5)
        return both.contiguous().reshape(-1)

    @staticmethod
    def split_grid(cost, G: int):
        S = len(cost)
        n = [1] * S
        for _ in range(max(0, G - S)):
            i = max(range(S), key=lambda j: cost[j] / n[j])
            n[i] += 1
        pre = [0]
        for v in n:
            pre.append(pre[-1] + v)
        return pre, pre[-1]


def tp_fused_fwd(fw: FusedTPWeights, x: torch.Tensor, y: torch.Tensor, h: torch.Tensor, edge_src: torch.Tensor,
                 csr: EdgeCSR, want_w: bool):
    _require_cuda(x, y, h, edge_src)
    plan = fw.plan
    if csr.perm is not None:
        raise RuntimeError("tp_fused_fwd: edges must be grouped by destination (no permutation)")
    if x.dtype != torch.float32 or y.dtype != torch.float32 or h.dtype != torch.float32:
        raise TypeError("tp_fused_fwd: float32 only")
    N, E = x.shape[0], edge_src.numel()
    if x.shape[1] != plan.d_in or tuple(y.shape) != (E, plan.s_dim) or h.shape[0] != E or h.shape[1] != fw.K:
        raise ValueError("tp_fused_fwd: shape mismatch")
    x, y, h = x.contiguous(), y.contiguous(), h.contiguous()
    out = torch.empty((N, plan.d_out), dtype=torch.float32, device=x.device)
    w = torch.empty((E, plan.weight_numel), dtype=torch.float32, device=x.device) if want_w else None
    _capi.check(
        _capi.lib().nqb_tp_fused_fwd(plan.handle, _ptr(x), _ptr(y), _ptr(h), h.stride(0), fw.K, _ptr(fw.prepared),
                                     _ptr(csr.row_ptr), _ptr(edge_src), N, E, _ptr(out), _ptr(w), _ptr(fw.cta0_dev),
                                     int(fw.nctas), _stream()),
        "nqb_tp_fused_fwd",
    )
    return out, w


_DETERMINISTIC = os.environ.get("NQB_DETERMINISTIC", "0") not in ("", "0")


def set_deterministic(on: bool = True) -> None:
    global _DETERMINISTIC
    _DETERMINISTIC = bool(on)


def deterministic() -> bool:
    return _DETERMINISTIC or torch.are_deterministic_algorithms_enabled()


class _SrcCSRCache:

    def __init__(self):
        self._tls = threading.local()

    def get(self, edge_src: torch.Tensor, num_nodes: int):
        key = (edge_src.data_ptr(), edge_src.numel(), edge_src._version, num_nodes, edge_src.device)
        ent = getattr(self._tls, "ent", None)
        if ent is not None and ent[0] == key:
            return ent[1], ent[2]
        keys, perm = torch.sort(edge_src, stable=True)
        seg = torch.empty(num_nodes + 1, dtype=torch.int64, device=edge_src.device)
        _capi.check(_capi.lib().nqb_csr_from_sorted(_ptr(keys.contiguous()), edge_src.numel(), num_nodes, _ptr(seg), _stream()),
                    "nqb_csr_from_sorted")
        self._tls.ent = (key, perm.contiguous(), seg, edge_src)
        return self._tls.ent[1], seg

    def clear(self):
        self._tls.ent = None


src_csr_cache = _SrcCSRCache()


def tp_scatter_bwd_raw(plan: TPPlan, x, y, w, edge_src, csr: EdgeCSR, gout, need_x: bool = True,
                       force_deterministic: Optional[bool] = None):
    L = _capi.lib()
    N, E = x.shape[0], edge_src.numel()
    det = deterministic() if force_deterministic is None else bool(force_deterministic)
    gw = torch.empty_like(w)
    if N == 0 or E == 0:
        gw.zero_()
        return (torch.zeros_like(x) if need_x else None), torch.zeros_like(y), gw
    gout = gout.contiguous()
    dt = _DT[x.dtype]
    if not det:
        gx = torch.zeros_like(x) if need_x else None
        gy = torch.zeros_like(y)
        _capi.check(L.nqb_tp_scatter_bwd(plan.handle, dt, _ptr(x), _ptr(y), _ptr(w), _ptr(csr.row_ptr), _ptr(csr.perm),
                                         _ptr(edge_src), _ptr(gout), N, E, _ptr(gx), _ptr(gy), _ptr(gw), 0, _stream()),
                    "nqb_tp_scatter_bwd")
        return gx, gy, gw
    ns = int(L.nqb_tp_scatter_gy_slices(plan.handle, dt))
    if ns <= 0:
        raise RuntimeError("nequip_b200: this kernel library has no deterministic backward")
    gxe = torch.empty((E, x.shape[1]), dtype=x.dtype, device=x.device) if need_x else None
    gys = torch.zeros((ns, E, y.shape[1]), dtype=y.dtype, device=y.device)
    _capi.check(L.nqb_tp_scatter_bwd(plan.handle, dt, _ptr(x), _ptr(y), _ptr(w), _ptr(csr.row_ptr), _ptr(csr.perm),
                                     _ptr(edge_src), _ptr(gout), N, E, _ptr(gxe), _ptr(gys), _ptr(gw), 1, _stream()),
                "nqb_tp_scatter_bwd")
    gx = None
    if need_x:
        perm_t, seg_t = src_csr_cache.get(edge_src, N)
        gx = torch.empty_like(x)
        _capi.check(L.nqb_segment_sum(dt, _ptr(gxe), x.shape[1], _ptr(perm_t), _ptr(seg_t), N, _ptr(gx), _stream()),
                    "nqb_segment_sum")
    gy = gys[0]
    for q in range(1, ns):
        gy = gy + gys[q]
    return gx, gy, gw


class _SHFn(torch.autograd.Function):
    @staticmethod
    def forward(ctx, vec, lmax: int, out_dtype):
        L = _capi.lib()
        E = vec.shape[0]
        y = torch.empty((E, (lmax + 1) ** 2), dtype=out_dtype, device=vec.device)
        _capi.check(L.nqb_sh_fwd(lmax, _ptr(vec), E, _DT[out_dtype], _ptr(y), _stream()), "nqb_sh_fwd")
        ctx.lmax, ctx.out_dtype = lmax, out_dtype
        ctx.save_for_backward(vec)
        return y

    @staticmethod
    @torch.autograd.function.once_differentiable
    def backward(ctx, gy):
        (vec,) = ctx.saved_tensors
        L = _capi.lib()
        E = vec.shape[0]
        gvec = torch.empty_like(vec)
        gy = gy.to(ctx.out_dtype).contiguous()
        _capi.check(L.nqb_sh_bwd(ctx.lmax, _ptr(vec), E, _DT[ctx.out_dtype], _ptr(gy), _ptr(gvec), _stream()),
                    "nqb_sh_bwd")
        return gvec, None, None


def spherical_harmonics(vec: torch.Tensor, lmax: int, out_dtype=torch.float32) -> torch.Tensor:
    _require_cuda(vec)
    if vec.dim() != 2 or vec.shape[1] != 3:
        raise ValueError("vec must be [E, 3]")
    return _SHFn.apply(vec.double().contiguous(), int(lmax), out_dtype)


class _EdgeEmbedFn(torch.autograd.Function):
    @staticmethod
    def forward(ctx, pos, edge_index, shift, cell, lmax, num_bessel, r_max, poly_p, prefactor, out_dtype, sink=None):
        L = _capi.lib()
        N, E = pos.shape[0], edge_index.shape[1]
        dev = pos.device
        vec = torch.empty((E, 3), dtype=torch.float64, device=dev)
        y = torch.empty((E, (lmax + 1) ** 2), dtype=out_dtype, device=dev)
        emb = torch.empty((E, num_bessel), dtype=out_dtype, device=dev)
        _capi.check(
            L.nqb_edge_embed_fwd(lmax, num_bessel, r_max, poly_p, prefactor, _ptr(pos), _ptr(edge_index), _ptr(shift),
                                 _ptr(cell), N, E, _DT[out_dtype], _ptr(vec), _ptr(y), _ptr(emb), _stream()),
            "nqb_edge_embed_fwd",
        )
        ctx.args = (lmax, num_bessel, r_max, poly_p, prefactor, out_dtype, N)
        ctx.sink = sink
        ctx.save_for_backward(vec, edge_index)
        ctx.mark_non_differentiable(vec)
        return vec, y, emb

    @staticmethod
    @torch.autograd.function.once_differentiable
    def backward(ctx, _gvec, gy, gemb):
        vec, edge_index = ctx.saved_tensors
        lmax, num_bessel, r_max, poly_p, prefactor, out_dtype, N = ctx.args
        L = _capi.lib()
        E = vec.shape[0]
        gpos = torch.zeros((N, 3), dtype=torch.float64, device=vec.device)
        gy = None if gy is None else gy.to(out_dtype).contiguous()
        gemb = None if gemb is None else gemb.to(out_dtype).contiguous()
        gvec = torch.empty_like(vec) if ctx.sink is not None else None
        _capi.check(
            L.nqb_edge_embed_bwd(lmax, num_bessel, r_max, poly_p, prefactor, _ptr(vec), _ptr(edge_index), N, E,
                                 _DT[out_dtype], _ptr(gy), _ptr(gemb), _ptr(gpos), _ptr(gvec), _stream()),
            "nqb_edge_embed_bwd",
        )
        if ctx.sink is not None:
            ctx.sink["edge_vectors"], ctx.sink["edge_vector_grad"] = vec, gvec
        return gpos, None, None, None, None, None, None, None, None, None, None


class _EdgeEmbedVecFn(torch.autograd.Function):

    @staticmethod
    def forward(ctx, vec, lmax, num_bessel, r_max, poly_p, prefactor, out_dtype):
        L = _capi.lib()
        E = vec.shape[0]
        dev = vec.device
        pos = torch.cat([vec, torch.zeros((1, 3), dtype=torch.float64, device=dev)], 0)
        ar = torch.arange(E, dtype=torch.int64, device=dev)
        edge_index = torch.stack([torch.full_like(ar, E), ar]).contiguous()
        vec_out = torch.empty((E, 3), dtype=torch.float64, device=dev)
        y = torch.empty((E, (lmax + 1) ** 2), dtype=out_dtype, device=dev)
        emb = torch.empty((E, num_bessel), dtype=out_dtype, device=dev)
        _capi.check(
            L.nqb_edge_embed_fwd(lmax, num_bessel, r_max, poly_p, prefactor, _ptr(pos), _ptr(edge_index), 0, 0, E + 1, E,
                                 _DT[out_dtype], _ptr(vec_out), _ptr(y), _ptr(emb), _stream()),
            "nqb_edge_embed_fwd",
        )
        ctx.args = (lmax, num_bessel, r_max, poly_p, prefactor, out_dtype)
        ctx.save_for_backward(vec_out, edge_index)
        return y, emb

    @staticmethod
    @torch.autograd.function.once_differentiable
    def backward(ctx, gy, gemb):
        vec, edge_index = ctx.saved_tensors
        lmax, num_bessel, r_max, poly_p, prefactor, out_dtype = ctx.args
        E = vec.shape[0]
        gvec = torch.empty_like(vec)
        gy = None if gy is None else gy.to(out_dtype).contiguous()
        gemb = None if gemb is None else gemb.to(out_dtype).contiguous()
        _capi.check(
            _capi.lib().nqb_edge_embed_bwd(lmax, num_bessel, r_max, poly_p, prefactor, _ptr(vec), _ptr(edge_index), E + 1, E,
                                           _DT[out_dtype], _ptr(gy), _ptr(gemb), 0, _ptr(gvec), _stream()),
            "nqb_edge_embed_bwd",
        )
        return gvec, None, None, None, None, None, None


def edge_embed_from_vectors(vec, *, lmax: int, num_bessel: int = 8, r_max: float, poly_p: float = 6.0,
                            prefactor: float = 1.0, out_dtype=torch.float32):
    _require_cuda(vec)
    return _EdgeEmbedVecFn.apply(vec.double().contiguous(), int(lmax), int(num_bessel), float(r_max), float(poly_p),
                                 float(prefactor), out_dtype)


def edge_embed(pos, edge_index, shift=None, cell=None, *, lmax: int, num_bessel: int = 8, r_max: float,
               poly_p: float = 6.0, prefactor: float = 1.0, out_dtype=torch.float32, edge_grad_sink=None):
    _require_cuda(pos, edge_index)
    pos = pos.double().contiguous()
    edge_index = edge_index.long().contiguous()
    if (shift is None) != (cell is None):
        raise ValueError("shift and cell must be given together")
    if shift is not None:
        shift = shift.double().contiguous()
        cell = cell.double().reshape(3, 3).contiguous()
    return _EdgeEmbedFn.apply(pos, edge_index, shift, cell, int(lmax), int(num_bessel), float(r_max),
                              float(poly_p), float(prefactor), out_dtype, edge_grad_sink)


class _ZBLFn(torch.autograd.Function):
    @staticmethod
    def forward(ctx, geom, edge_index, shift, cell, types, table, r_max, poly_p, cutoff_f32, from_vectors, sink):
        N, E, T = types.numel(), edge_index.shape[1], table.shape[0]
        csr = csr_cache.get(edge_index[0], N)
        pos, vec = (None, geom) if from_vectors else (geom, None)
        e_atom = torch.empty((N, 1), dtype=torch.float64, device=types.device)
        _capi.check(
            _capi.lib().nqb_zbl_fwd(_ptr(pos), _ptr(edge_index), _ptr(shift), _ptr(cell), _ptr(vec), _ptr(types),
                                    _ptr(table), T, _ptr(csr.row_ptr), _ptr(csr.perm), N, E, r_max, poly_p,
                                    int(cutoff_f32), _ptr(e_atom), _stream()),
            "nqb_zbl_fwd",
        )
        ctx.args = (r_max, poly_p, cutoff_f32, from_vectors)
        ctx.sink = sink
        ctx.save_for_backward(geom, edge_index, shift, cell, types, table)
        return e_atom

    @staticmethod
    @torch.autograd.function.once_differentiable
    def backward(ctx, ge):
        geom, edge_index, shift, cell, types, table = ctx.saved_tensors
        r_max, poly_p, cutoff_f32, from_vectors = ctx.args
        N, E = types.numel(), edge_index.shape[1]
        pos, vec = (None, geom) if from_vectors else (geom, None)
        gpos = None if from_vectors else torch.zeros_like(geom)
        gvec = torch.empty((E, 3), dtype=torch.float64, device=geom.device) \
            if from_vectors or ctx.sink is not None else None
        ge = ge.to(torch.float64).contiguous()
        _capi.check(
            _capi.lib().nqb_zbl_bwd(_ptr(pos), _ptr(edge_index), _ptr(shift), _ptr(cell), _ptr(vec), _ptr(types),
                                    _ptr(table), table.shape[0], N, E, r_max, poly_p, int(cutoff_f32), _ptr(ge),
                                    _ptr(gpos), _ptr(gvec), _stream()),
            "nqb_zbl_bwd",
        )
        if ctx.sink is not None:
            ctx.sink["pair_edge_vector_grad"] = gvec
        return (gvec if from_vectors else gpos), None, None, None, None, None, None, None, None, None, None


def zbl_energy(pos, edge_index, types, table, *, shift=None, cell=None, edge_vectors=None, r_max: float,
               poly_p: float = 6.0, cutoff_dtype=torch.float64, edge_grad_sink=None):
    _require_cuda(edge_index, types, table)
    edge_index = edge_index.long().contiguous()
    types = types.view(-1).long().contiguous()
    table = table.to(torch.float64).contiguous()
    if table.dim() != 3 or table.shape[0] != table.shape[1] or table.shape[2] != 2:
        raise ValueError(f"zbl_energy: table must be [T, T, 2], got {tuple(table.shape)}")
    if cutoff_dtype not in (torch.float32, torch.float64):
        raise ValueError(f"zbl_energy: cutoff_dtype must be float32 or float64, got {cutoff_dtype}")
    if (pos is None) == (edge_vectors is None):
        raise ValueError("zbl_energy: give exactly one of pos and edge_vectors")
    if (shift is None) != (cell is None):
        raise ValueError("shift and cell must be given together")
    if edge_vectors is not None:
        _require_cuda(edge_vectors)
        if shift is not None:
            raise ValueError("zbl_energy: edge_vectors already include the cell shifts")
        geom, from_vectors = edge_vectors.double().contiguous(), True
    else:
        _require_cuda(pos)
        geom, from_vectors = pos.double().contiguous(), False
        if geom.shape != (types.numel(), 3):
            raise ValueError(f"zbl_energy: pos must be [{types.numel()}, 3], got {tuple(geom.shape)}")
        if shift is not None:
            shift = shift.double().contiguous()
            cell = cell.double().reshape(3, 3).contiguous()
    return _ZBLFn.apply(geom, edge_index, shift, cell, types, table, float(r_max), float(poly_p),
                        cutoff_dtype == torch.float32, from_vectors, edge_grad_sink)


@dataclass
class GemmProblem:

    a_off: int
    lda: int
    c_off: int
    ldc: int
    B: torch.Tensor
    scale: float = 1.0
    transposed: bool = False
    accumulate: bool = False
    rs_off: int = -1
    skip_zero_rows: bool = False
    atomic: bool = False
    act: str = "none"


GEMM_ACT_FLAGS = {"none": 0, "silu": 8, "silu_save": 8 | 16, "silu_grad": 32}


class GroupedGemm:

    def __init__(self, problems, device):
        L = _capi.lib()
        self.problems = list(problems)
        rows = self.descriptor_rows(self.problems)
        blobs = []
        for p, row in zip(self.problems, rows):
            K, N = row[6], row[7]
            Bc = p.B.detach().to(device).contiguous()
            prep = torch.empty(int(L.nqb_gemm_prepared_floats(K, N)), dtype=torch.float32, device=device)
            _capi.check(L.nqb_gemm_prepare(_ptr(Bc), Bc.shape[1], K, N, int(p.transposed), float(p.scale), _ptr(prep),
                                           _stream()), "nqb_gemm_prepare")
            blobs.append(prep)
        self.act = any(p.act != "none" for p in self.problems)
        self.needs_aux = any(p.act in ("silu_save", "silu_grad") for p in self.problems)
        self.ntiles_total = rows[-1][10] + rows[-1][9]
        self.tile_ctas, self.sched_ctas = self._weighted_split(rows, device)
        self.prepared = torch.cat(blobs)
        self.descs = torch.tensor(rows, dtype=torch.int64, device=device)
        self.ndesc = len(rows)

    @staticmethod
    def descriptor_rows(problems) -> List[List[int]]:
        if not problems:
            raise ValueError("GroupedGemm: empty problem list")
        L = _capi.lib()
        rows, b_off, tile0 = [], 0, 0
        for p in problems:
            K, N = (p.B.shape[1], p.B.shape[0]) if p.transposed else (p.B.shape[0], p.B.shape[1])
            if any(v % 4 for v in (K, N, p.lda, p.ldc, p.a_off, p.c_off)):
                raise ValueError("GroupedGemm: K, N, lda, ldc and offsets must be multiples of 4")
            if p.B.dtype != torch.float32:
                raise TypeError("GroupedGemm: float32 only")
            if p.act not in GEMM_ACT_FLAGS:
                raise ValueError(f"GroupedGemm: unknown act {p.act!r} (one of {', '.join(GEMM_ACT_FLAGS)})")
            if p.act != "none" and (p.accumulate or p.atomic):
                raise ValueError("GroupedGemm: an activation cannot be combined with accumulate or atomic")
            kchunks, ntiles = (K + 31) // 32, (N + 127) // 128
            rows.append([p.a_off, p.c_off, b_off, p.rs_off, p.lda, p.ldc, K, N, kchunks, ntiles, tile0,
                         (1 if p.accumulate else 0) | (2 if p.skip_zero_rows else 0) | (4 if p.atomic else 0)
                         | GEMM_ACT_FLAGS[p.act]])
            b_off += int(L.nqb_gemm_prepared_floats(K, N))
            tile0 += ntiles
        return rows

    @staticmethod
    def _weighted_split(rows, device):
        if torch.device(device).type != "cuda":
            return None, 0
        G = torch.cuda.get_device_properties(device).multi_processor_count
        cost = []
        for (_a, _c, _b, _rs, _lda, _ldc, K, N, _kch, ntiles, _t0, flags) in rows:
            for t in range(ntiles):
                ncols = min(128, N - t * 128)
                cost.append(((K + 31) // 32) * 1000.0 + ((ncols + 31) // 32) * 650.0 * (2.0 if flags & 5 else 1.0))
        T = len(cost)
        if T > G or T < 2 or max(cost) < 1.3 * min(cost):
            return None, 0
        n = [1] * T
        for _ in range(G - T):
            i = max(range(T), key=lambda j: cost[j] / n[j])
            n[i] += 1
        tab, c0 = [], 0
        for j in range(T):
            tab += [c0, n[j]]
            c0 += n[j]
        return torch.tensor(tab, dtype=torch.int32, device=device), c0

    def run(self, a: torch.Tensor, c: torch.Tensor, M: int, rowscale: Optional[torch.Tensor] = None,
            aux: Optional[torch.Tensor] = None):
        _require_cuda(a, c)
        if a.dtype != torch.float32 or c.dtype != torch.float32:
            raise TypeError("GroupedGemm.run: float32 only")
        rs_ld = int(rowscale.shape[-1]) if rowscale is not None else 0
        if not self.act:
            if aux is not None:
                raise ValueError("GroupedGemm.run: aux given, but no problem sets an activation")
            _capi.check(
                _capi.lib().nqb_gemm_grouped(_ptr(self.descs), self.ndesc, self.ntiles_total, _ptr(self.tile_ctas),
                                             int(self.sched_ctas), _ptr(a), _ptr(self.prepared), _ptr(c),
                                             _ptr(rowscale), rs_ld, int(M), _stream()),
                "nqb_gemm_grouped",
            )
            return c
        if self.needs_aux and aux is None:
            raise ValueError("GroupedGemm.run: silu_save / silu_grad problems need aux")
        if aux is not None:
            _require_cuda(aux)
            if aux.dtype != torch.float32:
                raise TypeError("GroupedGemm.run: float32 only")
        _capi.check(
            _capi.lib().nqb_gemm_grouped_act(_ptr(self.descs), self.ndesc, self.ntiles_total, _ptr(self.tile_ctas),
                                             int(self.sched_ctas), _ptr(a), _ptr(self.prepared), _ptr(c),
                                             _ptr(rowscale), rs_ld, int(M), _ptr(c if aux is None else aux), _stream()),
            "nqb_gemm_grouped_act",
        )
        return c


def mlp_hidden_fwd(emb: torch.Tensor, w1s: torch.Tensor, h: torch.Tensor, h_lo=None) -> None:
    if h_lo is not None:
        raise ValueError("mlp_hidden_fwd: h_lo must be None")
    _require_cuda(emb, w1s, h)
    _capi.check(_capi.lib().nqb_mlp_hidden_fwd(_ptr(emb), _ptr(w1s), emb.shape[0], emb.shape[1], w1s.shape[1], _ptr(h),
                                               _stream()), "nqb_mlp_hidden_fwd")


def mlp_hidden_variant(variant: int = 0) -> int:
    if variant not in (0, 2):
        raise ValueError(f"mlp_hidden_variant: only variant 2 exists, got {variant!r}")
    return 2


def mlp_hidden_bwd(emb: torch.Tensor, w1s: torch.Tensor, gh: torch.Tensor, gemb: torch.Tensor) -> None:
    _require_cuda(emb, w1s, gh, gemb)
    _capi.check(_capi.lib().nqb_mlp_hidden_bwd(_ptr(emb), _ptr(w1s), _ptr(gh), emb.shape[0], emb.shape[1], w1s.shape[1],
                                               _ptr(gemb), _stream()), "nqb_mlp_hidden_bwd")


class GateTables:

    def __init__(self, irreps_scalars, irreps_gates, irreps_gated, layout: str, device):
        from .irreps import Irreps

        sc, ga, gd = Irreps(irreps_scalars), Irreps(irreps_gates), Irreps(irreps_gated)
        if sum(m for m, _ in ga) != sum(m for m, _ in gd):
            raise ValueError("Gate: one gate per gated multiplicity")
        ns, ng = sc.dim, ga.dim
        self.d_in = ns + ng + gd.dim
        self.d_out = ns + gd.dim
        src, gate, kind = [0] * self.d_out, [-1] * self.d_out, [0] * self.d_out
        tab = [[0] * 6 for _ in range(self.d_in)]
        off = 0
        for mul, ir in sc:
            k = 0 if ir.p == 1 else 1
            for u in range(mul):
                src[off + u], kind[off + u] = off + u, k
                tab[off + u] = [0, off + u, 0, 0, 0, k]
            off += mul
        gate_kind = []
        for mul, ir in ga:
            gate_kind += [0 if ir.p == 1 else 1] * mul
        g0, in_off, out_off = 0, ns + ng, ns
        for mul, ir in gd:
            d = ir.dim
            stride = mul if layout == "ir_mul" else 1
            for u in range(mul):
                gcol, k = ns + g0 + u, gate_kind[g0 + u]
                first = u if layout == "ir_mul" else u * d
                tab[gcol] = [2, out_off + first, in_off + first, stride, d, k]
                for c in range(d):
                    pos = first + c * stride
                    src[out_off + pos], gate[out_off + pos], kind[out_off + pos] = in_off + pos, gcol, k
                    tab[in_off + pos] = [1, out_off + pos, gcol, 0, 0, k]
            g0 += mul
            in_off += mul * d
            out_off += mul * d
        mk = lambda v: torch.tensor(v, dtype=torch.int32, device=device).contiguous()
        self.src, self.gate, self.kind = mk(src), mk(gate), mk(kind)
        self.tab = mk([x for row in tab for x in row])


class _GateFn(torch.autograd.Function):
    @staticmethod
    def forward(ctx, x, tabs: GateTables):
        x = x.contiguous()
        out = torch.empty((x.shape[0], tabs.d_out), dtype=x.dtype, device=x.device)
        _capi.check(_capi.lib().nqb_gate_fwd(_DT[x.dtype], _ptr(x), x.shape[0], tabs.d_in, tabs.d_out, _ptr(tabs.src),
                                             _ptr(tabs.gate), _ptr(tabs.kind), _ptr(out), _stream()), "nqb_gate_fwd")
        ctx.tabs = tabs
        ctx.save_for_backward(x)
        return out

    @staticmethod
    @torch.autograd.function.once_differentiable
    def backward(ctx, gout):
        (x,) = ctx.saved_tensors
        gout = gout.contiguous()
        gx = torch.empty_like(x)
        t = ctx.tabs
        _capi.check(_capi.lib().nqb_gate_bwd(_DT[x.dtype], _ptr(x), _ptr(gout), x.shape[0], t.d_in, t.d_out, _ptr(t.tab),
                                             _ptr(gx), _stream()), "nqb_gate_bwd")
        return gx, None


def gate(x: torch.Tensor, tabs: GateTables) -> torch.Tensor:
    _require_cuda(x)
    if x.dtype not in _DT or x.dim() != 2 or x.shape[1] != tabs.d_in:
        raise ValueError("gate: x must be [N, %d] float32/float64" % tabs.d_in)
    return _GateFn.apply(x, tabs)


def _nl_cell(cell, pbc):
    import numpy as np

    if isinstance(pbc, bool):
        pbc = (pbc,) * 3
    pbc = [bool(b) for b in (pbc.tolist() if torch.is_tensor(pbc) else pbc)]
    if cell is None:
        if any(pbc):
            raise ValueError("Periodic boundary conditions requested but no cell was provided.")
        cell_np = np.eye(3)
    else:
        cell_np = (cell.detach().cpu().double().reshape(3, 3).numpy() if torch.is_tensor(cell) else np.asarray(cell, dtype=np.float64).reshape(3, 3)).copy()
    return pbc, cell_np, np.linalg.inv(cell_np)


class _NlArgs:

    def __init__(self, N: int, cell_np, inv_np, pbc, r_max: float, lo, width, nb=None):
        import numpy as np

        perp = 1.0 / np.linalg.norm(inv_np, axis=0)
        fixed = nb is not None
        nb, sr = ([int(n) for n in nb] if fixed else [1, 1, 1]), [1, 1, 1]
        cap = max(1, int(round((4 * max(N, 1)) ** (1.0 / 3.0))))
        for d in range(3):
            extent = perp[d] * (1.0 if pbc[d] else width[d])
            if not fixed:
                nb[d] = int(min(cap, max(1, np.floor(extent / r_max))))
            sr[d] = int(np.ceil(r_max / (extent / nb[d]) - 1e-12)) if pbc[d] else 1
            sr[d] = max(sr[d], 1)
        I3 = C.c_int * 3
        D9, D3 = C.c_double * 9, C.c_double * 3
        self.cell, self.inv = D9(*cell_np.reshape(-1)), D9(*inv_np.reshape(-1))
        self.pbc, self.nb, self.sr = I3(*[int(b) for b in pbc]), I3(*nb), I3(*sr)
        self.lo, self.width = D3(*lo), D3(*width)
        self.r_max = float(r_max)
        self.nbins = nb[0] * nb[1] * nb[2]


def _nl_scratch(N: int, nbins: int, dev) -> Dict[str, torch.Tensor]:
    return {
        "wpos": torch.empty((N, 3), dtype=torch.float64, device=dev),
        "base": torch.empty((N, 3), dtype=torch.int32, device=dev),
        "cidx": torch.empty((N, 3), dtype=torch.int32, device=dev),
        "binid": torch.empty((N,), dtype=torch.int64, device=dev),
        "sorted_bin": torch.empty((N,), dtype=torch.int64, device=dev),
        "order": torch.empty((N,), dtype=torch.int64, device=dev),
        "bins": torch.arange(nbins + 1, device=dev, dtype=torch.int64),
        "bin_start": torch.empty((nbins + 1,), dtype=torch.int64, device=dev),
        "counts": torch.zeros((N,), dtype=torch.int64, device=dev),
        "row_ptr": torch.zeros((N + 1,), dtype=torch.int64, device=dev),
    }


def _nl_rows(pos: torch.Tensor, a: _NlArgs, s: Dict[str, torch.Tensor],
             params_dev: Optional[torch.Tensor] = None) -> None:
    L = _capi.lib()
    N = pos.shape[0]
    st = _stream()
    if params_dev is None:
        _capi.check(L.nqb_nl_bin(_ptr(pos), N, a.cell, a.inv, a.pbc, a.nb, a.sr, a.lo, a.width, a.r_max,
                                 _ptr(s["wpos"]), _ptr(s["base"]), _ptr(s["binid"]), _ptr(s["cidx"]), st), "nqb_nl_bin")
    else:
        _capi.check(L.nqb_nl_bin_dp(_ptr(pos), N, _ptr(params_dev), _ptr(s["wpos"]), _ptr(s["base"]), _ptr(s["binid"]),
                                    _ptr(s["cidx"]), st), "nqb_nl_bin_dp")
    torch.sort(s["binid"], stable=True, out=(s["sorted_bin"], s["order"]))
    torch.searchsorted(s["sorted_bin"], s["bins"], out=s["bin_start"])
    if params_dev is None:
        _capi.check(L.nqb_nl_count(N, a.cell, a.inv, a.pbc, a.nb, a.sr, a.r_max, _ptr(s["wpos"]), _ptr(s["cidx"]),
                                   _ptr(s["order"]), _ptr(s["bin_start"]), _ptr(s["counts"]), st), "nqb_nl_count")
    else:
        _capi.check(L.nqb_nl_count_dp(N, _ptr(params_dev), _ptr(s["wpos"]), _ptr(s["cidx"]), _ptr(s["order"]),
                                      _ptr(s["bin_start"]), _ptr(s["counts"]), st), "nqb_nl_count_dp")
    torch.cumsum(s["counts"], 0, out=s["row_ptr"][1:])


def neighbor_list(pos: torch.Tensor, cell=None, pbc=True, r_max: float = 5.0, transpose_perm: bool = False):
    import numpy as np

    _require_cuda(pos)
    L = _capi.lib()
    pos = pos.detach().double().contiguous()
    N = pos.shape[0]
    dev = pos.device
    pbc, cell_np, inv_np = _nl_cell(cell, pbc)
    lo = np.zeros(3)
    width = np.ones(3)
    if not all(pbc) and N > 0:
        frac = pos @ torch.as_tensor(inv_np, device=dev)
        fmin, fmax = frac.min(0).values.cpu().numpy(), frac.max(0).values.cpu().numpy()
        for d in range(3):
            if not pbc[d]:
                lo[d], width[d] = fmin[d], max(fmax[d] - fmin[d], 1e-9) * (1 + 1e-9)
    a = _NlArgs(N, cell_np, inv_np, pbc, r_max, lo, width)
    s = _nl_scratch(N, a.nbins, dev)
    _nl_rows(pos, a, s)
    row_ptr = s["row_ptr"]
    E = int(row_ptr[-1].item())
    edge_index = torch.empty((2, E), dtype=torch.int64, device=dev)
    shifts = torch.empty((E, 3), dtype=torch.float64, device=dev)
    _capi.check(L.nqb_nl_fill(N, E, a.cell, a.inv, a.pbc, a.nb, a.sr, a.r_max, _ptr(s["wpos"]), _ptr(s["cidx"]),
                              _ptr(s["base"]), _ptr(s["order"]), _ptr(s["bin_start"]), _ptr(row_ptr), _ptr(edge_index),
                              _ptr(shifts), _stream()), "nqb_nl_fill")
    out = {"edge_index": edge_index, "edge_cell_shift": shifts, "row_ptr": row_ptr}
    if transpose_perm:
        out["edge_transpose_perm"] = torch.argsort(edge_index[1] * N + edge_index[0], stable=True)
    return out


def null_edge_shift(cell, r_max: float):
    import numpy as np

    cell_np = (cell.detach().cpu().double().reshape(3, 3).numpy() if torch.is_tensor(cell)
               else np.asarray(cell, dtype=np.float64).reshape(3, 3))
    lengths = np.linalg.norm(cell_np, axis=1)
    d = int(np.argmax(lengths))
    shift = np.zeros(3)
    shift[d] = np.floor(r_max / lengths[d]) + 2
    return shift


def _nl_cell_block(cell, r_max: float, nb, num_atoms: int):
    import numpy as np

    c = cell.detach().cpu().double().numpy() if torch.is_tensor(cell) else np.asarray(cell, dtype=np.float64)
    if c.shape not in ((3, 3), (1, 3, 3)):
        raise ValueError(f"set_cell: cell must be [3, 3] or [1, 3, 3], got {tuple(c.shape)}")
    c = c.reshape(3, 3)
    if not np.all(np.isfinite(c)):
        raise ValueError("set_cell: cell is not finite")
    vol = abs(float(np.linalg.det(c)))
    if not vol > 1e-12 * float(np.prod(np.linalg.norm(c, axis=1))):
        raise ValueError("set_cell: cell is singular")
    pbc, cell_np, inv_np = _nl_cell(c, True)
    a = _NlArgs(num_atoms, cell_np, inv_np, pbc, r_max, np.zeros(3), np.ones(3), nb=nb)
    pad_shift = null_edge_shift(cell_np, r_max)
    L = _capi.lib()
    block = C.create_string_buffer(int(L.nqb_nl_params_bytes()))
    _capi.check(L.nqb_nl_params_pack(a.cell, a.inv, a.pbc, a.nb, a.sr, a.r_max, (C.c_double * 3)(*pad_shift), block),
                "nqb_nl_params_pack")
    return a, pad_shift, block


class NeighborListPlan:

    def __init__(self, num_atoms: int, cell, pbc, r_max: float, capacity: int, device=None,
                 variable_cell: bool = False):
        import numpy as np

        if cell is None:
            raise ValueError("NeighborListPlan needs a cell")
        if isinstance(pbc, bool):
            pbc = (pbc,) * 3
        pbc = [bool(b) for b in (pbc.tolist() if torch.is_tensor(pbc) else pbc)]
        if len(pbc) != 3 or not all(pbc):
            raise ValueError("NeighborListPlan needs all three directions periodic (the bounding box of a "
                             "non-periodic direction is found on the host at every call); use a large periodic box")
        if int(num_atoms) < 1 or int(capacity) < 0:
            raise ValueError("NeighborListPlan needs num_atoms >= 1 and capacity >= 0")
        self.num_atoms, self.capacity, self.r_max = int(num_atoms), int(capacity), float(r_max)
        pbc, cell_np, inv_np = _nl_cell(cell, pbc)
        self.pad_shift = null_edge_shift(cell_np, r_max)
        self._pad_shift_c = (C.c_double * 3)(*self.pad_shift)
        dev = torch.device(device) if device is not None else (
            cell.device if torch.is_tensor(cell) and cell.is_cuda else torch.device("cuda"))
        self.device = dev
        self._a = _NlArgs(self.num_atoms, cell_np, inv_np, pbc, r_max, np.zeros(3), np.ones(3))
        self._s = _nl_scratch(self.num_atoms, self._a.nbins, dev)
        N, cap = self.num_atoms, self.capacity
        self.edge_index = torch.empty((2, cap), dtype=torch.int64, device=dev)
        self.edge_cell_shift = torch.empty((cap, 3), dtype=torch.float64, device=dev)
        self.row_ptr = torch.empty((N + 1,), dtype=torch.int64, device=dev)
        self.num_edges = torch.empty((1,), dtype=torch.int64, device=dev)
        self.overflow = torch.empty((1,), dtype=torch.int32, device=dev)
        self.variable_cell = bool(variable_cell)
        self._params_dev = None
        if self.variable_cell:
            self.nbins = tuple(self._a.nb)
            nbytes = int(_capi.lib().nqb_nl_params_bytes())
            self._params_dev = torch.empty((nbytes,), dtype=torch.uint8, device=dev)
            self._params_host = torch.empty((nbytes,), dtype=torch.uint8).pin_memory()
            self._params_event: Optional[torch.cuda.Event] = None
            self.set_cell(cell)

    def set_cell(self, cell) -> None:
        if not self.variable_cell:
            raise ValueError("NeighborListPlan.set_cell needs a plan built with variable_cell=True")
        a, pad_shift, block = _nl_cell_block(cell, self.r_max, self.nbins, self.num_atoms)
        if self._params_event is not None:
            self._params_event.synchronize()
        C.memmove(self._params_host.data_ptr(), block, len(block))
        with torch.cuda.device(self.device):
            self._params_dev.copy_(self._params_host, non_blocking=True)
            self._params_event = torch.cuda.Event()
            self._params_event.record()
        self._a, self.pad_shift = a, pad_shift

    def run(self, pos: torch.Tensor) -> Dict[str, torch.Tensor]:
        _require_cuda(pos)
        if tuple(pos.shape) != (self.num_atoms, 3):
            raise ValueError(f"NeighborListPlan: pos must be [{self.num_atoms}, 3], got {tuple(pos.shape)}")
        pos = pos.detach().double().contiguous()
        L = _capi.lib()
        a, s = self._a, self._s
        _nl_rows(pos, a, s, self._params_dev)
        st = _stream()
        _capi.check(L.nqb_nl_pad(self.num_atoms, self.capacity, _ptr(s["row_ptr"]), _ptr(self.row_ptr),
                                 _ptr(self.num_edges), _ptr(self.overflow), st), "nqb_nl_pad")
        if self.variable_cell:
            _capi.check(L.nqb_nl_fill_capacity_dp(self.num_atoms, self.capacity, _ptr(self._params_dev),
                                                  _ptr(s["wpos"]), _ptr(s["cidx"]), _ptr(s["base"]), _ptr(s["order"]),
                                                  _ptr(s["bin_start"]), _ptr(self.row_ptr), _ptr(self.overflow),
                                                  _ptr(self.edge_index), _ptr(self.edge_cell_shift), st),
                        "nqb_nl_fill_capacity_dp")
        else:
            _capi.check(L.nqb_nl_fill_capacity(self.num_atoms, self.capacity, a.cell, a.inv, a.pbc, a.nb, a.sr, a.r_max,
                                               _ptr(s["wpos"]), _ptr(s["cidx"]), _ptr(s["base"]), _ptr(s["order"]),
                                               _ptr(s["bin_start"]), _ptr(self.row_ptr), _ptr(self.overflow),
                                               self._pad_shift_c, _ptr(self.edge_index), _ptr(self.edge_cell_shift),
                                               st),
                        "nqb_nl_fill_capacity")
        for t in (self.edge_index, self.edge_cell_shift, self.row_ptr, self.num_edges, self.overflow):
            torch.autograd.graph.increment_version(t)
        return {"edge_index": self.edge_index, "edge_cell_shift": self.edge_cell_shift, "row_ptr": self.row_ptr,
                "num_edges": self.num_edges, "overflow": self.overflow}
```

Baseline: 375,300.

## Deduplicate reverse edge pairs so the radial MLP runs once per pair

Adds a pass that finds, for each edge, its reverse edge (swapped endpoints, negated shift, bitwise-identical radial embedding) using the CSR, then compacts one representative row per pair. The radial MLP hidden layer and the grouped GEMM then run only over the representative rows, and the GEMM epilogue scatters each result to both edges of the pair. This is meant to roughly halve the radial MLP FLOPs, at the cost of extra pairing kernels and a data-dependent row count read on the device. Correctness relies on exact bitwise equality of the embeddings, so an edge without a matching partner is simply computed on its own.

```diff
diff --git a/include/nqb.h b/include/nqb.h
--- a/include/nqb.h
+++ b/include/nqb.h
@@ -116,6 +116,13 @@
 int nqb_mlp_hidden_bwd(const float* emb, const float* W1s, const float* grad_h, int64_t E, int num_bessel,
                        int hidden, float* grad_emb, nqb_stream_t st);
 
+int64_t nqb_edge_pairs_work_size(int64_t E);
+int nqb_edge_pairs(const int64_t* edge_index, int64_t E, int64_t N, const double* shift, const float* emb,
+                   int num_bessel, const int64_t* row_ptr, const int64_t* perm, int64_t* work, int64_t* pair_rows,
+                   int64_t* count, nqb_stream_t st);
+int nqb_mlp_hidden_fwd_rows(const float* emb, const float* W1s, const int64_t* pair_rows, const int64_t* count,
+                            int64_t capacity, int num_bessel, int hidden, float* h, nqb_stream_t st);
+
 int64_t nqb_gemm_prepared_floats(int K, int N);
 int nqb_gemm_prepare(const float* B, int64_t ldb, int K, int N, int transposed, float scale, float* prepared,
                      nqb_stream_t st);
@@ -125,6 +132,9 @@
 int nqb_gemm_grouped_act(const void* descs_dev, int ndesc, int ntiles_total, const int32_t* tile_ctas_dev,
                          int sched_ctas, const float* a_base, const float* prepared_base, float* c_base,
                          const float* rowscale_base, int64_t rs_ld, int64_t M, float* aux_base, nqb_stream_t st);
+int nqb_gemm_grouped_pairs(const void* descs_dev, int ndesc, int ntiles_total, const int32_t* tile_ctas_dev,
+                           int sched_ctas, const float* a_base, const float* prepared_base, float* c_base,
+                           const int64_t* pair_rows, const int64_t* count_dev, int64_t capacity, nqb_stream_t st);
 
 int nqb_gate_fwd(int dtype, const void* x, int64_t N, int d_in, int d_out, const int32_t* src,
                  const int32_t* gate, const int32_t* kind, void* out, nqb_stream_t st);
diff --git a/nequip_b200/_capi.py b/nequip_b200/_capi.py
--- a/nequip_b200/_capi.py
+++ b/nequip_b200/_capi.py
@@ -63,12 +63,16 @@
         _i32, [_vp, _vp, _vp, _vp, _vp, _vp, _vp, _i32, _i64, _i64, _dbl, _dbl, _i32, _vp, _vp, _vp, _vp]),
     "nqb_mlp_hidden_fwd": (_i32, [_vp, _vp, _i64, _i32, _i32, _vp, _vp]),
     "nqb_mlp_hidden_bwd": (_i32, [_vp, _vp, _vp, _i64, _i32, _i32, _vp, _vp]),
+    "nqb_mlp_hidden_fwd_rows": (_i32, [_vp, _vp, _vp, _vp, _i64, _i32, _i32, _vp, _vp]),
+    "nqb_edge_pairs_work_size": (_i64, [_i64]),
+    "nqb_edge_pairs": (_i32, [_vp, _i64, _i64, _vp, _vp, _i32, _vp, _vp, _vp, _vp, _vp, _vp]),
     "nqb_gemm_prepared_floats": (_i64, [_i32, _i32]),
     "nqb_gemm_prepare": (_i32, [_vp, _i64, _i32, _i32, _i32, C.c_float, _vp, _vp]),
     "nqb_gate_fwd": (_i32, [_i32, _vp, _i64, _i32, _i32, _vp, _vp, _vp, _vp, _vp]),
     "nqb_gate_bwd": (_i32, [_i32, _vp, _vp, _i64, _i32, _i32, _vp, _vp, _vp]),
     "nqb_gemm_grouped": (_i32, [_vp, _i32, _i32, _vp, _i32, _vp, _vp, _vp, _vp, _i64, _i64, _vp]),
     "nqb_gemm_grouped_act": (_i32, [_vp, _i32, _i32, _vp, _i32, _vp, _vp, _vp, _vp, _i64, _i64, _vp, _vp]),
+    "nqb_gemm_grouped_pairs": (_i32, [_vp, _i32, _i32, _vp, _i32, _vp, _vp, _vp, _vp, _vp, _i64, _vp]),
 }
 
 
diff --git a/nequip_b200/csrc/nqb_gemm.cu b/nequip_b200/csrc/nqb_gemm.cu
--- a/nequip_b200/csrc/nqb_gemm.cu
+++ b/nequip_b200/csrc/nqb_gemm.cu
@@ -78,14 +78,16 @@
 
 __device__ __forceinline__ void bar_wg(int wg) { asm volatile("bar.sync %0, 128;" ::"r"(1 + wg) : "memory"); }
 
-template <bool ACT>
+template <bool ACT, bool PAIRS = false>
 __global__ void __launch_bounds__(NTHREADS, 1)
 k_gemm3x(const GemmDesc* __restrict__ descs, int ndesc, int ntiles_total, const int32_t* __restrict__ tile_ctas,
          int sched_ctas, const float* __restrict__ a_base, const float* __restrict__ b_base, float* __restrict__ c_base,
-         const float* __restrict__ rs_base, int64_t rs_ld, int64_t M, float* __restrict__ aux_base) {
+         const float* __restrict__ rs_base, int64_t rs_ld, int64_t M, float* __restrict__ aux_base,
+         const int64_t* __restrict__ m_dev, const int64_t* __restrict__ pair_rows) {
   extern __shared__ __align__(1024) uint8_t smem_raw[];
   Smem& S = *reinterpret_cast<Smem*>(smem_raw);
   const int tid = threadIdx.x, wg = tid >> 7, warp = (tid >> 5) & 3, lane = tid & 31;
+  if constexpr (PAIRS) M = min(M, *m_dev);
   const int64_t mtiles = (M + TM - 1) / TM;
 
   if (tid == 0) {
@@ -239,6 +241,24 @@
         }
       }
       const int64_t m0 = mt * TM + wg * MW + r0;
+      if constexpr (PAIRS) {
+#pragma unroll
+        for (int half = 0; half < 2; ++half) {
+          const int64_t m = m0 + half * 8;
+          if (m >= M) continue;
+          const longlong2 pr = __ldg(reinterpret_cast<const longlong2*>(pair_rows) + m);
+          float* crow0 = C + pr.x * ldc + c0;
+          float* crow1 = C + pr.y * ldc + c0;
+#pragma unroll
+          for (int j = 0; j < TN / 8; ++j) {
+            if (j * 8 + c0 < w.ncols) {
+              const float2 v = make_float2(hh[4 * j + 2 * half], hh[4 * j + 2 * half + 1]);
+              *reinterpret_cast<float2*>(crow0 + j * 8) = v;
+              if (pr.y >= 0) *reinterpret_cast<float2*>(crow1 + j * 8) = v;
+            }
+          }
+        }
+      } else
 #pragma unroll
       for (int half = 0; half < 2; ++half) {
         const int64_t m = m0 + half * 8;
@@ -341,11 +361,12 @@
   return 0;
 }
 
-template <bool ACT>
+template <bool ACT, bool PAIRS = false>
 static int gemm_grouped_launch(const char* who, const void* descs_dev, int ndesc, int ntiles_total,
                                const int32_t* tile_ctas_dev, int sched_ctas, const float* a_base,
                                const float* prepared_base, float* c_base, float* aux_base, const float* rowscale_base,
-                               int64_t rs_ld, int64_t M, nqb_stream_t st) {
+                               int64_t rs_ld, int64_t M, nqb_stream_t st, const int64_t* m_dev = nullptr,
+                               const int64_t* pair_rows = nullptr) {
   auto fail = [&](const char* what) {
     char msg[160];
     snprintf(msg, sizeof(msg), "%s: %s", who, what);
@@ -356,13 +377,16 @@
   if (M == 0) return 0;
   if (!descs_dev || !a_base || !prepared_base || !c_base) return fail("null pointer");
   if (ACT && !aux_base) return fail("aux_base is null (bit4 / bit5 problems store to or read from it)");
+  if (PAIRS && (!m_dev || !pair_rows)) return fail("pair_rows or count is null");
+  if (PAIRS && ((uintptr_t)pair_rows & 15)) return fail("pair_rows must be 16-byte aligned");
   if (((uintptr_t)a_base | (uintptr_t)prepared_base | (uintptr_t)c_base | (uintptr_t)aux_base) & 15)
     return fail(ACT ? "a_base, prepared_base, c_base and aux_base must be 16-byte aligned"
                     : "a_base, prepared_base and c_base must be 16-byte aligned");
   static bool attr_set[64] = {false};
   const int dev = gemm_device();
   if (!attr_set[dev]) {
-    cudaError_t e = cudaFuncSetAttribute(k_gemm3x<ACT>, cudaFuncAttributeMaxDynamicSharedMemorySize, (int)sizeof(Smem) + 1024);
+    cudaError_t e = cudaFuncSetAttribute(k_gemm3x<ACT, PAIRS>, cudaFuncAttributeMaxDynamicSharedMemorySize,
+                                         (int)sizeof(Smem) + 1024);
     if (e != cudaSuccess) return nqb_set_error(cudaGetErrorString(e));
     attr_set[dev] = true;
   }
@@ -370,9 +394,9 @@
   int grid = (int)(nwork < gemm_sm_count() ? nwork : gemm_sm_count());
   if (tile_ctas_dev != nullptr && sched_ctas > 0 && sched_ctas <= gemm_sm_count()) grid = sched_ctas;
   else tile_ctas_dev = nullptr;
-  k_gemm3x<ACT><<<grid, NTHREADS, sizeof(Smem) + 1024, (cudaStream_t)st>>>(
+  k_gemm3x<ACT, PAIRS><<<grid, NTHREADS, sizeof(Smem) + 1024, (cudaStream_t)st>>>(
       (const GemmDesc*)descs_dev, ndesc, ntiles_total, tile_ctas_dev, sched_ctas, a_base, prepared_base, c_base,
-      rowscale_base, rs_ld, M, aux_base);
+      rowscale_base, rs_ld, M, aux_base, m_dev, pair_rows);
   nqb_count_launch();
   cudaError_t e = cudaGetLastError();
   if (e != cudaSuccess) return nqb_set_error(cudaGetErrorString(e));
@@ -393,3 +417,12 @@
   return gemm_grouped_launch<true>("nqb_gemm_grouped_act", descs_dev, ndesc, ntiles_total, tile_ctas_dev, sched_ctas,
                                    a_base, prepared_base, c_base, aux_base, rowscale_base, rs_ld, M, st);
 }
+
+extern "C" int nqb_gemm_grouped_pairs(const void* descs_dev, int ndesc, int ntiles_total, const int32_t* tile_ctas_dev,
+                                      int sched_ctas, const float* a_base, const float* prepared_base, float* c_base,
+                                      const int64_t* pair_rows, const int64_t* count_dev, int64_t capacity,
+                                      nqb_stream_t st) {
+  return gemm_grouped_launch<false, true>("nqb_gemm_grouped_pairs", descs_dev, ndesc, ntiles_total, tile_ctas_dev,
+                                          sched_ctas, a_base, prepared_base, c_base, nullptr, nullptr, 0, capacity,
+                                          st, count_dev, pair_rows);
+}
diff --git a/nequip_b200/csrc/nqb_mlp.cu b/nequip_b200/csrc/nqb_mlp.cu
--- a/nequip_b200/csrc/nqb_mlp.cu
+++ b/nequip_b200/csrc/nqb_mlp.cu
@@ -21,6 +21,16 @@
   }
   return r;
 }
+template <bool ROWS>
+__device__ __forceinline__ Basis8 load_slot(const float* __restrict__ emb, const int64_t* __restrict__ rows, int64_t u,
+                                            int64_t n) {
+  if constexpr (ROWS) {
+    const int64_t e = u < n ? __ldg(rows + 2 * u) : 0;
+    return load_basis(emb, e, u < n ? e + 1 : 0);
+  } else {
+    return load_basis(emb, u, n);
+  }
+}
 __device__ __forceinline__ void bcast_basis(const Basis8& mine, int j, float (&x)[NB]) {
   x[0] = __shfl_sync(0xffffffffu, mine.a.x, j); x[1] = __shfl_sync(0xffffffffu, mine.a.y, j);
   x[2] = __shfl_sync(0xffffffffu, mine.a.z, j); x[3] = __shfl_sync(0xffffffffu, mine.a.w, j);
@@ -39,9 +49,13 @@
   }
 }
 
+template <bool ROWS = false>
 __global__ void __launch_bounds__(256) k_hidden_fwd(const float* __restrict__ emb, const float* __restrict__ W1s,
-                                                    int64_t E, float* __restrict__ h) {
+                                                    int64_t E, float* __restrict__ h,
+                                                    const int64_t* __restrict__ rows = nullptr,
+                                                    const int64_t* __restrict__ count = nullptr) {
   const int lane = threadIdx.x & 31, m0 = lane * 4;
+  if constexpr (ROWS) E = min(E, *count);
   float2 w01[NB], w23[NB];
 #pragma unroll
   for (int k = 0; k < NB; ++k) {
@@ -52,10 +66,10 @@
   const int64_t nwarps = (int64_t)gridDim.x * (blockDim.x >> 5);
   const int64_t nbatch = (E + 31) >> 5;
   int64_t b = (int64_t)blockIdx.x * (blockDim.x >> 5) + (threadIdx.x >> 5);
-  Basis8 cur = load_basis(emb, b * 32 + lane, b < nbatch ? E : 0);
+  Basis8 cur = load_slot<ROWS>(emb, rows, b * 32 + lane, b < nbatch ? E : 0);
   for (; b < nbatch; b += nwarps) {
     const int64_t bn = b + nwarps;
-    const Basis8 nxt = load_basis(emb, bn * 32 + lane, bn < nbatch ? E : 0);
+    const Basis8 nxt = load_slot<ROWS>(emb, rows, bn * 32 + lane, bn < nbatch ? E : 0);
     const int64_t e0 = b * 32;
     const int cnt = (int)((E - e0) < 32 ? (E - e0) : 32);
     float* hrow = h + e0 * H + m0;
@@ -140,6 +154,127 @@
   }
 }
 
+constexpr int PT = 1024;
+
+__global__ void __launch_bounds__(256) k_pair_candidates(const int64_t* __restrict__ ei, int64_t E, int64_t N,
+                                                         const double* __restrict__ shift,
+                                                         const uint32_t* __restrict__ emb, int words,
+                                                         const int64_t* __restrict__ row_ptr,
+                                                         const int64_t* __restrict__ perm, int64_t* __restrict__ cand) {
+  const int lane = threadIdx.x & 31, g = lane >> 3, r = lane & 7;
+  const int64_t nwarps = (int64_t)gridDim.x * (blockDim.x >> 5);
+  for (int64_t wv = (int64_t)blockIdx.x * (blockDim.x >> 5) + (threadIdx.x >> 5); wv * 4 < E; wv += nwarps) {
+    const int64_t e = wv * 4 + g;
+    int64_t a = -1, s = 0, s1 = 0;
+    if (e < E) {
+      a = ei[e];
+      const int64_t b = ei[E + e];
+      if (b >= 0 && b < N) {
+        s = row_ptr[b];
+        s1 = row_ptr[b + 1];
+      }
+    }
+    int64_t found = -1;
+    bool done = s >= s1;
+    while (__any_sync(0xffffffffu, !done)) {
+      int64_t f = -1;
+      bool hit = false;
+      if (!done && s + r < s1) {
+        f = perm ? perm[s + r] : s + r;
+        hit = f != e && ei[E + f] == a;
+        if (hit && shift)
+          hit = shift[3 * f] == -shift[3 * e] && shift[3 * f + 1] == -shift[3 * e + 1] &&
+                shift[3 * f + 2] == -shift[3 * e + 2];
+        for (int k = 0; hit && k < words; ++k) hit = emb[f * words + k] == emb[e * words + k];
+      }
+      const uint32_t grp = (__ballot_sync(0xffffffffu, hit) >> (8 * g)) & 0xffu;
+      const int64_t first = __shfl_sync(0xffffffffu, f, 8 * g + (grp ? __ffs(grp) - 1 : 0));
+      if (!done && grp) {
+        found = first;
+        done = true;
+      }
+      s += 8;
+      if (s >= s1) done = true;
+    }
+    if (r == 0 && e < E) cand[e] = found;
+  }
+}
+
+__device__ __forceinline__ int pair_rep(const int64_t* __restrict__ cand, int64_t e, int64_t* partner) {
+  const int64_t c = cand[e];
+  const int64_t p = (c >= 0 && cand[c] == e) ? c : -1;
+  *partner = p;
+  return (p < 0 || e < p) ? 1 : 0;
+}
+
+__device__ __forceinline__ int block_scan256(int v, int* scratch, int* total) {
+  const int lane = threadIdx.x & 31, warp = threadIdx.x >> 5;
+#pragma unroll
+  for (int o = 1; o < 32; o <<= 1) {
+    const int t = __shfl_up_sync(0xffffffffu, v, o);
+    if (lane >= o) v += t;
+  }
+  if (lane == 31) scratch[warp] = v;
+  __syncthreads();
+  int before = 0, all = 0;
+#pragma unroll
+  for (int w = 0; w < 8; ++w) {
+    const int x = scratch[w];
+    before += (w < warp) ? x : 0;
+    all += x;
+  }
+  __syncthreads();
+  *total = all;
+  return v + before;
+}
+
+__global__ void __launch_bounds__(256) k_pair_block_counts(const int64_t* __restrict__ cand, int64_t E,
+                                                           int64_t* __restrict__ counts) {
+  __shared__ int scratch[8];
+  const int64_t e0 = (int64_t)blockIdx.x * PT + threadIdx.x * 4;
+  int n = 0;
+  int64_t p;
+#pragma unroll
+  for (int k = 0; k < 4; ++k)
+    if (e0 + k < E) n += pair_rep(cand, e0 + k, &p);
+  int total;
+  block_scan256(n, scratch, &total);
+  if (threadIdx.x == 0) counts[blockIdx.x] = total;
+}
+
+__global__ void __launch_bounds__(256) k_pair_write(const int64_t* __restrict__ cand, int64_t E,
+                                                    const int64_t* __restrict__ counts, int64_t* __restrict__ pair_rows,
+                                                    int64_t* __restrict__ count) {
+  __shared__ int scratch[8];
+  __shared__ int64_t base_part[8];
+  int64_t before = 0;
+  for (int64_t t = threadIdx.x; t < blockIdx.x; t += blockDim.x) before += counts[t];
+#pragma unroll
+  for (int o = 16; o > 0; o >>= 1) before += __shfl_xor_sync(0xffffffffu, before, o);
+  if ((threadIdx.x & 31) == 0) base_part[threadIdx.x >> 5] = before;
+  __syncthreads();
+  int64_t base = 0;
+#pragma unroll
+  for (int w = 0; w < 8; ++w) base += base_part[w];
+  const int64_t e0 = (int64_t)blockIdx.x * PT + threadIdx.x * 4;
+  int rep[4], n = 0;
+  int64_t partner[4];
+#pragma unroll
+  for (int k = 0; k < 4; ++k) {
+    rep[k] = (e0 + k < E) ? pair_rep(cand, e0 + k, &partner[k]) : 0;
+    n += rep[k];
+  }
+  int total;
+  int64_t u = base + block_scan256(n, scratch, &total) - n;
+#pragma unroll
+  for (int k = 0; k < 4; ++k)
+    if (rep[k]) {
+      reinterpret_cast<longlong2*>(pair_rows)[u] = make_longlong2(e0 + k, partner[k]);
+      ++u;
+    }
+  if (threadIdx.x == 0 && blockIdx.x == gridDim.x - 1) *count = base + total;
+}
+
 }
 
 extern "C" int nqb_set_error(const char* msg);
@@ -147,7 +282,7 @@
 
 template <typename K>
 static unsigned hidden_grid(K kernel, int which, int64_t E) {
-  static int ctas_dev[2][64] = {{0}, {0}};
+  static int ctas_dev[3][64] = {{0}, {0}, {0}};
   int dev = 0;
   cudaGetDevice(&dev);
   dev &= 63;
@@ -167,7 +302,23 @@
   if (E < 0) return nqb_set_error("nqb_mlp_hidden_fwd: negative size");
   if (E == 0) return 0;
   if (!emb || !W1s || !h) return nqb_set_error("nqb_mlp_hidden_fwd: null pointer");
-  k_hidden_fwd<<<hidden_grid(k_hidden_fwd, 0, E), 256, 0, (cudaStream_t)st>>>(emb, W1s, E, h);
+  k_hidden_fwd<<<hidden_grid(k_hidden_fwd<false>, 0, E), 256, 0, (cudaStream_t)st>>>(emb, W1s, E, h);
+  nqb_count_launch();
+  cudaError_t e = cudaGetLastError();
+  if (e != cudaSuccess) return nqb_set_error(cudaGetErrorString(e));
+  return 0;
+}
+
+extern "C" int nqb_mlp_hidden_fwd_rows(const float* emb, const float* W1s, const int64_t* pair_rows,
+                                       const int64_t* count, int64_t capacity, int num_bessel, int hidden, float* h,
+                                       nqb_stream_t st) {
+  if (num_bessel != NB || hidden != H)
+    return nqb_set_error("nqb_mlp_hidden_fwd_rows: only num_bessel=8, hidden=128 is built");
+  if (capacity < 0) return nqb_set_error("nqb_mlp_hidden_fwd_rows: negative size");
+  if (capacity == 0) return 0;
+  if (!emb || !W1s || !pair_rows || !count || !h) return nqb_set_error("nqb_mlp_hidden_fwd_rows: null pointer");
+  k_hidden_fwd<true><<<hidden_grid(k_hidden_fwd<true>, 2, capacity), 256, 0, (cudaStream_t)st>>>(emb, W1s, capacity, h,
+                                                                                                 pair_rows, count);
   nqb_count_launch();
   cudaError_t e = cudaGetLastError();
   if (e != cudaSuccess) return nqb_set_error(cudaGetErrorString(e));
@@ -186,3 +337,35 @@
   if (e != cudaSuccess) return nqb_set_error(cudaGetErrorString(e));
   return 0;
 }
+
+extern "C" int64_t nqb_edge_pairs_work_size(int64_t E) { return E > 0 ? E + (E + PT - 1) / PT : 0; }
+
+extern "C" int nqb_edge_pairs(const int64_t* edge_index, int64_t E, int64_t N, const double* shift, const float* emb,
+                              int num_bessel, const int64_t* row_ptr, const int64_t* perm, int64_t* work,
+                              int64_t* pair_rows, int64_t* count, nqb_stream_t st) {
+  if (E < 0 || N < 0 || num_bessel <= 0) return nqb_set_error("nqb_edge_pairs: bad size");
+  if (!count) return nqb_set_error("nqb_edge_pairs: null pointer");
+  if (E == 0) {
+    cudaError_t e = cudaMemsetAsync(count, 0, sizeof(int64_t), (cudaStream_t)st);
+    return e == cudaSuccess ? 0 : nqb_set_error(cudaGetErrorString(e));
+  }
+  if (!edge_index || !emb || !row_ptr || !work || !pair_rows) return nqb_set_error("nqb_edge_pairs: null pointer");
+  if ((uintptr_t)pair_rows & 15) return nqb_set_error("nqb_edge_pairs: pair_rows must be 16-byte aligned");
+  const int64_t tiles = (E + PT - 1) / PT;
+  int sms = 0, dev = 0;
+  cudaGetDevice(&dev);
+  cudaDeviceGetAttribute(&sms, cudaDevAttrMultiProcessorCount, dev);
+  const int64_t warps = (E + 3) / 4, cap = (int64_t)(sms > 0 ? sms : 132) * 8;
+  const unsigned cblocks = (unsigned)((warps + 7) / 8 < cap ? (warps + 7) / 8 : cap);
+  k_pair_candidates<<<cblocks, 256, 0, (cudaStream_t)st>>>(edge_index, E, N, shift,
+                                                            reinterpret_cast<const uint32_t*>(emb), num_bessel, row_ptr,
+                                                            perm, work);
+  nqb_count_launch();
+  k_pair_block_counts<<<(unsigned)tiles, 256, 0, (cudaStream_t)st>>>(work, E, work + E);
+  nqb_count_launch();
+  k_pair_write<<<(unsigned)tiles, 256, 0, (cudaStream_t)st>>>(work, E, work + E, pair_rows, count);
+  nqb_count_launch();
+  cudaError_t e = cudaGetLastError();
+  if (e != cudaSuccess) return nqb_set_error(cudaGetErrorString(e));
+  return 0;
+}
diff --git a/nequip_b200/nn/dense.py b/nequip_b200/nn/dense.py
--- a/nequip_b200/nn/dense.py
+++ b/nequip_b200/nn/dense.py
@@ -119,11 +119,16 @@
 
 class _RadialMLPGemmFn(torch.autograd.Function):
     @staticmethod
-    def forward(ctx, emb, mlp: "RadialMLPGemm", need_bwd: bool):
+    def forward(ctx, emb, mlp: "RadialMLPGemm", need_bwd: bool, pairs):
         E = emb.shape[0]
         out = torch.empty((E, mlp.W), dtype=emb.dtype, device=emb.device)
         pre = [] if need_bwd else None
-        mlp.fwd.run(mlp.hidden(emb, pre), out, E)
+        if pairs is not None and mlp.shares_pairs:
+            h = torch.empty((E, mlp.w1s.shape[1]), dtype=emb.dtype, device=emb.device)
+            ops.mlp_hidden_fwd_rows(emb, mlp.w1s, pairs, h)
+            mlp.fwd.run_pairs(h, out, pairs)
+        else:
+            mlp.fwd.run(mlp.hidden(emb, pre), out, E)
         ctx.mlp = mlp
         if need_bwd:
             ctx.save_for_backward(emb, *pre)
@@ -133,7 +138,7 @@
     @torch.autograd.function.once_differentiable
     def backward(ctx, gw):
         emb, *pre = ctx.saved_tensors
-        return ctx.mlp.grad_emb(emb, gw, pre), None, None
+        return ctx.mlp.grad_emb(emb, gw, pre), None, None, None
 
 
 class RadialMLPGemm:
@@ -151,6 +156,7 @@
         self.bwd = gemm(plan["bwd"])
         self._hidden = [(gemm(save), gemm(plain), save.B.shape[1]) for save, plain in plan["hidden"]]
         self._chain = [(self.bwd if p is plan["bwd"] else gemm(p), width, pre) for p, width, pre in plan["chain"]]
+        self.shares_pairs = self._hidden_kernel and not self._hidden
 
     @staticmethod
     def uses_hidden_kernel(first) -> bool:
@@ -217,8 +223,8 @@
             return gemb
         return g
 
-    def __call__(self, emb):
-        return _RadialMLPGemmFn.apply(emb.contiguous(), self, torch.is_grad_enabled() and emb.requires_grad)
+    def __call__(self, emb, pairs: Optional[Tuple[torch.Tensor, torch.Tensor]] = None):
+        return _RadialMLPGemmFn.apply(emb.contiguous(), self, torch.is_grad_enabled() and emb.requires_grad, pairs)
 
 
 class _FusedRadialTPFn(torch.autograd.Function):
diff --git a/nequip_b200/nn/model.py b/nequip_b200/nn/model.py
--- a/nequip_b200/nn/model.py
+++ b/nequip_b200/nn/model.py
@@ -289,7 +289,7 @@
     def _edge_weights(self, edge_embedding):
         return self.edge_mlp(edge_embedding)
 
-    def _use_fused(self, tc, edge_embedding, x, edge_attrs, edge_index) -> bool:
+    def _use_fused(self, tc, edge_embedding, x, edge_attrs, edge_index, pairs=None) -> bool:
         mode = self.use_fused_radial_tp
         if mode is True or mode is False:
             return mode
@@ -310,7 +310,7 @@
 
                 xd, yd, ed = x.detach(), edge_attrs.detach(), edge_embedding.detach()
                 tf = t(lambda: tc["fused"](ed, xd, yd, edge_index[0], edge_index[1]))
-                tu = t(lambda: self.tp_scatter(x=xd, edge_attr=yd, edge_weight=tc["mlp"](ed), edge_dst=edge_index[0],
+                tu = t(lambda: self.tp_scatter(x=xd, edge_attr=yd, edge_weight=tc["mlp"](ed, pairs), edge_dst=edge_index[0],
                                                edge_src=edge_index[1]))
             self._fused_choice = bool(tf < tu)
             self.fused_timing_ms = {"fused": tf, "unfused": tu}
@@ -329,7 +329,7 @@
                           f"wgmma kernels: {reason}", RuntimeWarning, stacklevel=3)
 
     def forward(self, x, node_attrs, edge_attrs, edge_embedding, edge_index, types=None, type_table=None,
-                n_own: Optional[int] = None, halo=None):
+                n_own: Optional[int] = None, halo=None, pairs=None):
         if n_own is not None and not self.is_first_layer:
             x = x[:n_own]
             node_attrs = node_attrs[:n_own]
@@ -340,7 +340,7 @@
             x = tc["lin1"](x) if self.norm_shortcut else tc["lin1"](x, self.norm_const.view(-1)[types].view(1, -1).contiguous())
             if halo is not None and not self.is_first_layer:
                 x = halo(x)
-            if tc["fused"] is not None and self._use_fused(tc, edge_embedding, x, edge_attrs, edge_index):
+            if tc["fused"] is not None and self._use_fused(tc, edge_embedding, x, edge_attrs, edge_index, pairs):
                 y = tc["fused"](edge_embedding, x, edge_attrs, edge_index[0], edge_index[1])
                 if y is not None:
                     x = y
@@ -351,7 +351,7 @@
                         x = tc["sc"](x_in, types, x)
                     return x
             if tc["mlp"] is not None:
-                w = tc["mlp"](edge_embedding)
+                w = tc["mlp"](edge_embedding, pairs)
             else:
                 self._note_fallback("radial MLP shape not supported by the grouped GEMM (needs at least one hidden "
                                     "layer, num_bessels and widths multiples of 4)")
@@ -433,8 +433,8 @@
         self.irreps_out = layer_out
 
     def forward(self, x, node_attrs, edge_attrs, edge_embedding, edge_index, types=None, type_table=None,
-                n_own=None, halo=None):
-        x = self.conv(x, node_attrs, edge_attrs, edge_embedding, edge_index, types, type_table, n_own, halo)
+                n_own=None, halo=None, pairs=None):
+        x = self.conv(x, node_attrs, edge_attrs, edge_embedding, edge_index, types, type_table, n_own, halo, pairs)
         return self.equivariant_nonlin(x)
 
 
@@ -534,6 +534,14 @@
             layer.conv.strict_fast_path = bool(on)
         return self
 
+    def _edge_pairs(self, edge_index, shift, edge_embedding, num_nodes):
+        if not (self.num_bessels == 8 and self.config["radial_mlp_depth"] == 1 and self.config["radial_mlp_width"] == 128
+                and edge_embedding.dtype == torch.float32 and self.node_layout == "ir_mul"):
+            return None
+        dst = edge_index[0]
+        csr = ops.csr_cache.get(dst if dst.dtype == torch.int64 else dst.long().contiguous(), num_nodes)
+        return ops.edge_pairs(edge_index, shift, edge_embedding, csr)
+
     @staticmethod
     def _reduce_energy(e_atom: torch.Tensor, data: Dict[str, torch.Tensor]) -> torch.Tensor:
         batch = data.get(BATCH_KEY)
@@ -567,8 +575,9 @@
             _vec, edge_attrs, edge_embedding = ops.edge_embed(
                 pos, edge_index, shift, cell, lmax=self.l_max, num_bessel=self.num_bessels, r_max=self.r_max,
                 poly_p=self.poly_p, prefactor=pre, out_dtype=self.model_dtype, edge_grad_sink=sink)
+        pairs = self._edge_pairs(edge_index, None if EDGE_VECTORS_KEY in data else shift, edge_embedding, types.numel())
         for layer in self.layers:
-            x = layer(x, node_attrs, edge_attrs, edge_embedding, edge_index, types, self.type_embed.weight)
+            x = layer(x, node_attrs, edge_attrs, edge_embedding, edge_index, types, self.type_embed.weight, pairs=pairs)
         e_atom = self.readout(x).to(torch.float64)
         if self.scales.numel():
             e_atom = e_atom * self.scales[types]
@@ -596,8 +605,10 @@
         _vec, edge_attrs, edge_embedding = ops.edge_embed(
             pos, edge_index, shift, cell, lmax=self.l_max, num_bessel=self.num_bessels, r_max=self.r_max,
             poly_p=self.poly_p, prefactor=(2 * math.pi) / (self.r_max * self.r_max), out_dtype=self.model_dtype)
+        pairs = self._edge_pairs(edge_index, shift, edge_embedding, types.numel())
         for layer in self.layers:
-            x = layer(x, node_attrs, edge_attrs, edge_embedding, edge_index, types, self.type_embed.weight, n_own, halo)
+            x = layer(x, node_attrs, edge_attrs, edge_embedding, edge_index, types, self.type_embed.weight, n_own, halo,
+                      pairs)
         e_atom = self.readout(x).to(torch.float64)
         t_own = types[:n_own]
         if self.scales.numel():
diff --git a/nequip_b200/ops.py b/nequip_b200/ops.py
--- a/nequip_b200/ops.py
+++ b/nequip_b200/ops.py
@@ -690,6 +690,55 @@
         )
         return c
 
+    def run_pairs(self, a: torch.Tensor, c: torch.Tensor, pairs: Tuple[torch.Tensor, torch.Tensor]):
+        pair_rows, count = pairs
+        _require_cuda(a, c, pair_rows, count)
+        if a.dtype != torch.float32 or c.dtype != torch.float32:
+            raise TypeError("GroupedGemm.run_pairs: float32 only")
+        if any(p.act != "none" or p.accumulate or p.atomic or p.skip_zero_rows or p.rs_off >= 0 for p in self.problems):
+            raise ValueError("GroupedGemm.run_pairs: plain problems only (no row scale, accumulate, atomic or activation)")
+        if pair_rows.dtype != torch.int64 or count.dtype != torch.int64 or pair_rows.dim() != 2 or pair_rows.shape[1] != 2:
+            raise ValueError("GroupedGemm.run_pairs: pair_rows must be [E, 2] and count [1], int64")
+        _capi.check(
+            _capi.lib().nqb_gemm_grouped_pairs(_ptr(self.descs), self.ndesc, self.ntiles_total, _ptr(self.tile_ctas),
+                                               int(self.sched_ctas), _ptr(a), _ptr(self.prepared), _ptr(c),
+                                               _ptr(pair_rows), _ptr(count), int(pair_rows.shape[0]), _stream()),
+            "nqb_gemm_grouped_pairs",
+        )
+        return c
+
+
+def edge_pairs(edge_index: torch.Tensor, shift: Optional[torch.Tensor], emb: torch.Tensor,
+               csr: EdgeCSR) -> Tuple[torch.Tensor, torch.Tensor]:
+    _require_cuda(edge_index, emb)
+    if emb.dtype != torch.float32 or emb.dim() != 2:
+        raise TypeError("edge_pairs: emb must be [E, num_bessel] float32")
+    edge_index = edge_index.long().contiguous()
+    E = edge_index.shape[1]
+    if emb.shape[0] != E or csr.num_edges != E:
+        raise ValueError("edge_pairs: emb / csr do not match edge_index")
+    emb = emb.contiguous()
+    if shift is not None:
+        shift = shift.double().contiguous()
+    L = _capi.lib()
+    dev = edge_index.device
+    pair_rows = torch.empty((E, 2), dtype=torch.int64, device=dev)
+    count = torch.empty(1, dtype=torch.int64, device=dev)
+    work = torch.empty(int(L.nqb_edge_pairs_work_size(E)), dtype=torch.int64, device=dev)
+    _capi.check(L.nqb_edge_pairs(_ptr(edge_index), E, csr.num_nodes, _ptr(shift), _ptr(emb), emb.shape[1],
+                                 _ptr(csr.row_ptr), _ptr(csr.perm), _ptr(work), _ptr(pair_rows), _ptr(count), _stream()),
+                "nqb_edge_pairs")
+    return pair_rows, count
+
+
+def mlp_hidden_fwd_rows(emb: torch.Tensor, w1s: torch.Tensor, pairs: Tuple[torch.Tensor, torch.Tensor],
+                        h: torch.Tensor) -> None:
+    pair_rows, count = pairs
+    _require_cuda(emb, w1s, pair_rows, count, h)
+    _capi.check(_capi.lib().nqb_mlp_hidden_fwd_rows(_ptr(emb), _ptr(w1s), _ptr(pair_rows), _ptr(count),
+                                                    pair_rows.shape[0], emb.shape[1], w1s.shape[1], _ptr(h), _stream()),
+                "nqb_mlp_hidden_fwd_rows")
+
 
 def mlp_hidden_fwd(emb: torch.Tensor, w1s: torch.Tensor, h: torch.Tensor, h_lo=None) -> None:
     if h_lo is not None:
```

Result: faster. 414,800 (median of 6 runs) (+10.5%).
